# pomonam/LearnablePoolingMethods

Hardware: AMD Instinct MI355X
Metric: clips/sec training step, NetVladV1 K=256 300-frame 1152-d, bs=80, 1/2/4/8 GPU (higher is better)
Workload: dtype f32

## Files before the change

include/lpm_hip.h:

```cpp
#ifndef LPM_HIP_H
#define LPM_HIP_H

#include <stddef.h>
#include <stdint.h>

#ifdef __cplusplus
extern "C" {
#endif

#define LPM_VERSION 100

typedef void* lpm_stream_t;

enum {
    LPM_OK = 0,
    LPM_ERR_BADARG = -1,
    LPM_ERR_UNSUPPORTED_SHAPE = -2,
    LPM_ERR_WORKSPACE = -3,
    LPM_ERR_LAUNCH = -4
};

enum {
    LPM_VLAD_SOFTMAX = 1,
    LPM_VLAD_RESIDUAL = 2,
    LPM_VLAD_OUT_KMAJOR = 4,
    LPM_VLAD_NRM_RAW = 8,
    LPM_VLAD_OUT_BF16 = 16,
    LPM_VLAD_TILES_BF16 = 32,
    LPM_VLAD_NRM_BF16 = 64,
    LPM_VLAD_RAW_KMAJOR = 128,
    LPM_VLAD_DEBUG_FALLBACK = 256,
    LPM_VLAD_WIDE_ALL = 512,
    LPM_VLAD_WIDE_NONE = 1024
};

int lpm_version(void);
const char* lpm_last_error(void);

void lpm_kernel_timing_enable(int on);
int lpm_k1_forms_disable(int mask);
int lpm_kernel_timing_read(int tag, float* ms, int max);

int lpm_clock_sampler(uint64_t* out, int n, int period_ticks, lpm_stream_t stream);
int lpm_clock_marker(uint64_t* out, int slot, lpm_stream_t stream);

int lpm_l2_normalize_rows(const float* x, int64_t rows, int F, float* y, lpm_stream_t stream);

int lpm_dequantize_l2_normalize(const unsigned char* q, const int32_t* num_frames, int B, int max_frames, int F,
                                float max_quantized_value, float min_quantized_value, float* y, lpm_stream_t stream);

size_t lpm_frame_stats_workspace_bytes(int B, int S, int F);
int lpm_frame_stats(const float* raw, const int32_t* num_frames, int B, int max_frames, int F, int S,
                    float* partial, lpm_stream_t stream);
int lpm_frame_apply(const float* raw, const int32_t* num_frames, int B, int max_frames, int F, int S,
                    const float* scale, const float* shift, float* y, lpm_stream_t stream);
int lpm_frame_apply_tiles(const float* raw, const int32_t* num_frames, int B, int max_frames, int F, int S,
                          const float* scale, const float* shift, float* y, void* xt_video, int Dv, void* xt_audio, int Da,
                          lpm_stream_t stream);
int lpm_frame_apply_tiles_split(const float* raw, const int32_t* num_frames, int B, int max_frames, int F, int S, const float* scale,
                                const float* shift, float* y_video, float* y_audio, void* xt_video, int Dv, void* xt_audio, int Da,
                                lpm_stream_t stream);
int lpm_frame_bn_bwd_split(const float* dy_video, int64_t ldv, const float* dy_audio, int64_t lda, int Dv, const float* raw,
                           const int32_t* num_frames, int B, int max_frames, int F, int S, const float* mean, const float* var, float eps,
                           float* dgamma, float* dbeta, void* workspace, size_t workspace_bytes, lpm_stream_t stream);
int lpm_frame_apply_tiles2(const float* raw, const int32_t* num_frames, int B, int max_frames, int F, int S,
                           const float* scale, const float* shift, float* y, void* xt_video, void* xr_video, int Dv,
                           void* xt_audio, void* xr_audio, int Da, lpm_stream_t stream);
int lpm_frame_stats_nblk(int B, int S);
int lpm_frame_inv_norm_q8(const unsigned char* q, const int32_t* num_frames, int B, int max_frames, int F, int S,
                          float max_quantized_value, float min_quantized_value, float* inv_norm, lpm_stream_t stream);
int lpm_frame_apply_q8(const unsigned char* q, const float* inv_norm, float max_quantized_value, float min_quantized_value,
                       const int32_t* num_frames, int B, int max_frames, int F, int S, const float* scale, const float* shift, float* y,
                       lpm_stream_t stream);
int lpm_frame_apply_tiles_q8(const unsigned char* q, const float* inv_norm, float max_quantized_value, float min_quantized_value,
                             const int32_t* num_frames, int B, int max_frames, int F, int S, const float* scale, const float* shift, float* y,
                             void* xt_video, int Dv, void* xt_audio, int Da, lpm_stream_t stream);
int lpm_frame_apply_tiles_split_q8(const unsigned char* q, const float* inv_norm, float max_quantized_value, float min_quantized_value,
                                   const int32_t* num_frames, int B, int max_frames, int F, int S, const float* scale, const float* shift,
                                   float* y_video, float* y_audio, void* xt_video, int Dv, void* xt_audio, int Da, lpm_stream_t stream);
int lpm_frame_apply_tiles2_q8(const unsigned char* q, const float* inv_norm, float max_quantized_value, float min_quantized_value,
                              const int32_t* num_frames, int B, int max_frames, int F, int S, const float* scale, const float* shift, float* y,
                              void* xt_video, void* xr_video, int Dv, void* xt_audio, void* xr_audio, int Da, lpm_stream_t stream);
int lpm_frame_apply_tiles_bf16_q8(const unsigned char* q, const float* inv_norm, float max_quantized_value, float min_quantized_value,
                                  const int32_t* num_frames, int B, int max_frames, int F, int S, const float* scale, const float* shift,
                                  float* y, void* xt_video, void* xr_video, int Dv, void* xt_audio, void* xr_audio, int Da,
                                  lpm_stream_t stream);
int lpm_frame_bn_bwd(const float* dy, int64_t lddy, const float* raw, const int32_t* num_frames, int B,
                     int max_frames, int F, int S, const float* mean, const float* var, float eps, float* dgamma,
                     float* dbeta, void* workspace, size_t workspace_bytes, lpm_stream_t stream);

int lpm_bn_fold(const float* partial, int nblk, int C, int64_t rows, const float* gamma, const float* beta,
                float eps, float decay, float* mean, float* var, float* scale, float* shift,
                float* moving_mean, float* moving_var, lpm_stream_t stream);

int lpm_assign_gemm_nblk(int M);
int lpm_assign_gemm_fwd(const float* x, int64_t ldx, const float* w, int M, int D, int K, int precision,
                        float* logits, float* partial, lpm_stream_t stream);

size_t lpm_row_tiles_bytes(int B, int T, int C);
size_t lpm_weight_tiles_bytes(int R, int N);
int lpm_assign_gemm_tiles_supported(int T, int D, int K);
int lpm_assign_gemm_tiles_nblk(int B, int T);
int lpm_split_rows_tiles(const float* x, int64_t ldx, int B, int T, int C, void* out, lpm_stream_t stream);
int lpm_split_weight_tiles(const float* w, int R, int N, int transposed, void* wt, lpm_stream_t stream);
int lpm_assign_gemm_tiles_fwd(const void* xr, const void* wt, int B, int T, int D, int K, float* logits, float* partial,
                              lpm_stream_t stream);
int lpm_assign_gemm_tiles_bwd_dx(const void* dlr, const void* wtt, int B, int T, int D, int K, float* dx, int64_t lddx,
                                 lpm_stream_t stream);
int lpm_dense_tiles_fwd(const void* xr, const void* wt, int M, int Kd, int N, float* y, int64_t ldo, int form, lpm_stream_t stream);
int lpm_dense_tiles_supported(int M, int Kd, int N);
int lpm_dense_tiles_act_image_fwd(const void* xr, const void* wt, const float* bias, int M, int Kd, int N, void* out3, lpm_stream_t stream);
size_t lpm_dense_tiles_relu_bwd_workspace_bytes(int M, int N);
int lpm_dense_tiles_relu_bwd_image(const void* dyr, const void* wtt, const void* act3, int M, int Kd, int N, void* out3, float* dbias,
                                   void* workspace, size_t workspace_bytes, lpm_stream_t stream);
int lpm_image_row_tiles(const void* x3, int M, int K, int order, void* out, lpm_stream_t stream);
int lpm_skinny_weight_grad_tiles(const void* xt, const void* dyt, int R, int N1, int N2, float* dw, lpm_stream_t stream);
size_t lpm_assign_gemm_tiles_bwd_dw_workspace_bytes(int B, int T, int D, int K);
int lpm_assign_gemm_tiles_bwd_dw(const void* xt, const void* dlt, int B, int T, int D, int K, float* dw, void* workspace,
                                 size_t workspace_bytes, lpm_stream_t stream);

int lpm_vlad_aggregate_fwd(const float* assign, const float* scale, const float* shift, const float* x,
                           int64_t ldx, const float* centres, int B, int T, int D, int K, int flags,
                           float* nrm, float* asum, float* colsq, float* csq, lpm_stream_t stream);
int lpm_vlad_finalize_fwd(const float* nrm, const float* csq, int B, int D, int K, int flags, float* out,
                          float* gsq, lpm_stream_t stream);

size_t lpm_xt_bytes(int B, int T, int D);
size_t lpm_at_bytes(int B, int T, int K);
int lpm_split_frames(const float* x, int64_t ldx, int B, int T, int D, void* xt, lpm_stream_t stream);
int lpm_assign_tiles(const float* assign, const float* scale, const float* shift, int B, int T, int K, int flags,
                     void* at, lpm_stream_t stream);
int lpm_vlad_aggregate_tiles_fwd(const void* at, const void* xt, const float* centres, int B, int T, int D, int K,
                                 int flags, float* nrm, float* asum, float* colsq, float* csq, lpm_stream_t stream);

int lpm_vlad_tiles3_supported(int D, int K);
int lpm_vlad_aggregate_tiles3_fwd(const void* at, const void* xt, const float* centres, int B, int T, int D, int K,
                                  int flags, float* nrm, float* asum, float* colsq_part, lpm_stream_t stream);
int lpm_vlad_finalize2_fwd(float* nrm, const float* colsq_part, int P, int B, int D, int K, int flags, float* out,
                           float* colsq, float* csq, float* gsq, lpm_stream_t stream);
int lpm_vlad_finalize2_fwd_ld(float* nrm, const float* colsq_part, int P, int B, int D, int K, int flags, float* out,
                              int64_t out_batch_stride, float* colsq, float* csq, float* gsq, lpm_stream_t stream);

int lpm_vlad_aggregate_raw_kmajor_fwd(const void* at, const void* xt, const float* centres, int B, int T, int D, int K, int flags,
                                      float* raw_kmajor, float* asum, float* colsq_part, lpm_stream_t stream);
int lpm_vlad_row_scales(const float* colsq_part, int P, int B, int K, float* scale, float* colsq, float* csq, float* gsq,
                        lpm_stream_t stream);
int lpm_vlad_clip_slabs(int D, int K);
int lpm_vlad_aggregate_clip_kmajor_fwd(const void* at, const void* xt, const float* centres, int B, int T, int D, int K, int flags,
                                       float* raw_kmajor, float* asum, float* colsq_part, lpm_stream_t stream);
int lpm_vlad_aggregate_clip_dmajor_fwd(const void* at, const void* xt, const float* centres, int B, int T, int D, int K, int flags,
                                       float* raw_dmajor, float* asum, float* colsq_part, lpm_stream_t stream);
// ... 295 lines not shown
```

learnablepoolingmethods_amd/_capi.py:

```python
from __future__ import annotations

import ctypes as C
import os
from typing import Optional

import torch

_HERE = os.path.dirname(os.path.abspath(__file__))
LIB_PATH = os.path.join(_HERE, "_lib", "liblpm_hip.so")

LPM_VLAD_SOFTMAX = 1
LPM_VLAD_RESIDUAL = 2
LPM_VLAD_OUT_KMAJOR = 4
LPM_VLAD_NRM_RAW = 8
LPM_VLAD_OUT_BF16 = 16
LPM_VLAD_TILES_BF16 = 32
LPM_VLAD_NRM_BF16 = 64
LPM_VLAD_RAW_KMAJOR = 128
LPM_VLAD_DEBUG_FALLBACK = 256
LPM_VLAD_WIDE_ALL = 512
LPM_VLAD_WIDE_NONE = 1024

_f = C.c_void_p
_i = C.c_int
_l = C.c_int64
_s = C.c_size_t
_fl = C.c_float
SIGNATURES = {
    "lpm_version": (_i, []),
    "lpm_last_error": (C.c_char_p, []),
    "lpm_kernel_timing_enable": (None, [_i]),
    "lpm_kernel_timing_read": (_i, [_i, C.POINTER(C.c_float), _i]),
    "lpm_clock_sampler": (_i, [_f, _i, _i, _f]),
    "lpm_clock_marker": (_i, [_f, _i, _f]),
    "lpm_l2_normalize_rows": (_i, [_f, _l, _i, _f, _f]),
    "lpm_dequantize_l2_normalize": (_i, [_f, _f, _i, _i, _i, _fl, _fl, _f, _f]),
    "lpm_frame_stats_workspace_bytes": (_s, [_i, _i, _i]),
    "lpm_frame_stats": (_i, [_f, _f, _i, _i, _i, _i, _f, _f]),
    "lpm_frame_apply": (_i, [_f, _f, _i, _i, _i, _i, _f, _f, _f, _f]),
    "lpm_frame_apply_tiles": (_i, [_f, _f, _i, _i, _i, _i, _f, _f, _f, _f, _i, _f, _i, _f]),
    "lpm_frame_apply_tiles_split": (_i, [_f, _f, _i, _i, _i, _i, _f, _f, _f, _f, _f, _i, _f, _i, _f]),
    "lpm_frame_stats_nblk": (_i, [_i, _i]),
    "lpm_frame_bn_bwd": (_i, [_f, _l, _f, _f, _i, _i, _i, _i, _f, _f, _fl, _f, _f, _f, _s, _f]),
    "lpm_frame_bn_bwd_split": (_i, [_f, _l, _f, _l, _i, _f, _f, _i, _i, _i, _i, _f, _f, _fl, _f, _f, _f, _s, _f]),
    "lpm_frame_inv_norm_q8": (_i, [_f, _f, _i, _i, _i, _i, _fl, _fl, _f, _f]),
    "lpm_frame_apply_q8": (_i, [_f, _f, _fl, _fl, _f, _i, _i, _i, _i, _f, _f, _f, _f]),
    "lpm_frame_apply_tiles_q8": (_i, [_f, _f, _fl, _fl, _f, _i, _i, _i, _i, _f, _f, _f, _f, _i, _f, _i, _f]),
    "lpm_frame_apply_tiles_split_q8": (_i, [_f, _f, _fl, _fl, _f, _i, _i, _i, _i, _f, _f, _f, _f, _f, _i, _f, _i, _f]),
    "lpm_frame_apply_tiles2_q8": (_i, [_f, _f, _fl, _fl, _f, _i, _i, _i, _i, _f, _f, _f, _f, _f, _i, _f, _f, _i, _f]),
    "lpm_frame_apply_tiles_bf16_q8": (_i, [_f, _f, _fl, _fl, _f, _i, _i, _i, _i, _f, _f, _f, _f, _f, _i, _f, _f, _i, _f]),
    "lpm_bn_fold": (_i, [_f, _i, _i, _l, _f, _f, _fl, _fl, _f, _f, _f, _f, _f, _f, _f]),
    "lpm_assign_gemm_nblk": (_i, [_i]),
    "lpm_assign_gemm_fwd": (_i, [_f, _l, _f, _i, _i, _i, _i, _f, _f, _f]),
    "lpm_row_tiles_bytes": (_s, [_i, _i, _i]),
    "lpm_weight_tiles_bytes": (_s, [_i, _i]),
    "lpm_assign_gemm_tiles_supported": (_i, [_i, _i, _i]),
    "lpm_assign_gemm_tiles_nblk": (_i, [_i, _i]),
    "lpm_split_rows_tiles": (_i, [_f, _l, _i, _i, _i, _f, _f]),
    "lpm_split_weight_tiles": (_i, [_f, _i, _i, _i, _f, _f]),
    "lpm_assign_gemm_tiles_fwd": (_i, [_f, _f, _i, _i, _i, _i, _f, _f, _f]),
    "lpm_assign_gemm_tiles_bwd_dx": (_i, [_f, _f, _i, _i, _i, _i, _f, _l, _f]),
    "lpm_dense_tiles_fwd": (_i, [_f, _f, _i, _i, _i, _f, _l, _i, _f]),
    "lpm_dense_tiles_supported": (_i, [_i, _i, _i]),
    "lpm_dense_tiles_act_image_fwd": (_i, [_f, _f, _f, _i, _i, _i, _f, _f]),
    "lpm_dense_tiles_relu_bwd_workspace_bytes": (_s, [_i, _i]),
    "lpm_dense_tiles_relu_bwd_image": (_i, [_f, _f, _f, _i, _i, _i, _f, _f, _f, _s, _f]),
    "lpm_image_row_tiles": (_i, [_f, _i, _i, _i, _f, _f]),
    "lpm_skinny_weight_grad_tiles": (_i, [_f, _f, _i, _i, _i, _f, _f]),
    "lpm_assign_gemm_tiles_bwd_dw_workspace_bytes": (_s, [_i, _i, _i, _i]),
    "lpm_assign_gemm_tiles_bwd_dw": (_i, [_f, _f, _i, _i, _i, _i, _f, _f, _s, _f]),
    "lpm_vlad_aggregate_fwd": (_i, [_f, _f, _f, _f, _l, _f, _i, _i, _i, _i, _i, _f, _f, _f, _f, _f]),
    "lpm_vlad_finalize_fwd": (_i, [_f, _f, _i, _i, _i, _i, _f, _f, _f]),
    "lpm_xt_bytes": (_s, [_i, _i, _i]),
    "lpm_at_bytes": (_s, [_i, _i, _i]),
    "lpm_split_frames": (_i, [_f, _l, _i, _i, _i, _f, _f]),
    "lpm_assign_tiles": (_i, [_f, _f, _f, _i, _i, _i, _i, _f, _f]),
    "lpm_vlad_aggregate_tiles_fwd": (_i, [_f, _f, _f, _i, _i, _i, _i, _i, _f, _f, _f, _f, _f]),
    "lpm_vlad_tiles3_supported": (_i, [_i, _i]),
    "lpm_vlad_aggregate_tiles3_fwd": (_i, [_f, _f, _f, _i, _i, _i, _i, _i, _f, _f, _f, _f]),
    "lpm_vlad_finalize2_fwd_ld": (_i, [_f, _f, _i, _i, _i, _i, _i, _f, _l, _f, _f, _f, _f]),
    "lpm_vlad_finalize2_fwd": (_i, [_f, _f, _i, _i, _i, _i, _i, _f, _f, _f, _f, _f]),
    "lpm_proj_supported": (_i, [_i, _l, _i]),
    "lpm_proj_fwd_workspace_bytes": (_s, [_i, _l, _i]),
    "lpm_proj_fwd": (_i, [_f, _l, _f, _i, _l, _i, _f, _f, _s, _f]),
    "lpm_proj_fwd_parts": (_i, [_f, _l, _l, _i, _f, _i, _f, _l, _f, _i, _l, _i, _f, _f, _s, _f]),
    "lpm_split_weight_tiles_parts": (_i, [_f, _l, _l, _i, _f, _i, _f, _l, _i, _l, _f, _f]),
    "lpm_proj_dx": (_i, [_f, _f, _i, _l, _i, _f, _l, _f]),
    "lpm_proj_fwd_parts_w16": (_i, [_f, _l, _l, _f, _i, _f, _l, _f, _i, _l, _i, _f, _f, _s, _f]),
    "lpm_proj_dx_w16": (_i, [_f, _f, _i, _l, _i, _f, _l, _f]),
    "lpm_frame_tiles_bf16_bytes": (_s, [_i, _i, _i]),
    "lpm_frame_steps_bf16": (_i, [_i]),
    "lpm_frame_apply_tiles2": (_i, [_f, _f, _i, _i, _i, _i, _f, _f, _f, _f, _f, _i, _f, _f, _i, _f]),
    "lpm_frame_apply_tiles_bf16": (_i, [_f, _f, _i, _i, _i, _i, _f, _f, _f, _f, _f, _i, _f, _f, _i, _f]),
    "lpm_split_weight_tiles_bf16": (_i, [_f, _i, _i, _i, _f, _f]),
    "lpm_split_frames_bf16": (_i, [_f, _l, _i, _i, _i, _f, _f]),
    "lpm_assign_gemm_tiles_fwd_bf16": (_i, [_f, _f, _i, _i, _i, _i, _f, _f, _f]),
    "lpm_k1_forms_disable": (_i, [_i]),
    "lpm_mha_bwd_set_terms": (_i, [_i]),
    "lpm_assign_gemm_tiles_bwd_dw_bf16": (_i, [_f, _f, _i, _i, _i, _i, _f, _f, _s, _f]),
    "lpm_assign_tiles_bf16": (_i, [_f, _f, _f, _i, _i, _i, _i, _f, _f]),
    "lpm_vlad_aggregate_tiles3_fwd_bf16": (_i, [_f, _f, _f, _i, _i, _i, _i, _i, _f, _f, _f, _f]),
    "lpm_vlad_clip16_slabs": (_i, [_i, _i]),
    "lpm_vlad_aggregate_clip_fwd_bf16": (_i, [_f, _f, _f, _i, _i, _i, _i, _i, _f, _f, _f, _f]),
    "lpm_vlad_aggregate_raw_kmajor_fwd": (_i, [_f, _f, _f, _i, _i, _i, _i, _i, _f, _f, _f, _f]),
    "lpm_vlad_smx_stats_bytes": (_s, [_i, _i]),
    "lpm_vlad_smx_supported": (_i, [_i, _i, _i]),
    "lpm_vlad_aggregate_raw_kmajor_smx_fwd": (_i, [_f, _f, _f, _f, _f, _i, _i, _i, _i, _i, _f, _f, _f, _f, _f]),
    "lpm_vlad_row_scales": (_i, [_f, _i, _i, _i, _f, _f, _f, _f, _f]),
    "lpm_vlad_clip_slabs": (_i, [_i, _i]),
    "lpm_vlad_aggregate_clip_kmajor_fwd": (_i, [_f, _f, _f, _i, _i, _i, _i, _i, _f, _f, _f, _f]),
    "lpm_vlad_aggregate_clip_dmajor_fwd": (_i, [_f, _f, _f, _i, _i, _i, _i, _i, _f, _f, _f, _f]),
    "lpm_vlad_kmajor_workspace_bytes": (_s, [_i, _i, _i]),
    "lpm_vlad_aggregate_kmajor_scaled_fwd": (_i, [_f, _f, _f, _i, _i, _i, _i, _i, _f, _f, _f, _f, _f, _f, _f, _s, _f]),
    "lpm_split_rows_scaled": (_i, [_f, _l, _l, _i, _f, _f, _f]),
    "lpm_layer_norm_act_fwd_rs": (_i, [_f, _f, _i, _f, _f, _f, _f, _i, _i, _i, _fl, _f, _l, _f, _f, _f, _s, _f]),
    "lpm_layer_norm_act_image_fwd": (_i, [_f, _f, _i, _f, _f, _f, _f, _i, _i, _i, _fl, _f, _l, _f, _f, _f, _f, _s, _f]),
    "lpm_vlad_fused_supported": (_i, [_i, _i]),
    "lpm_vlad_fused_workspace_bytes": (_s, [_i, _i, _i]),
    "lpm_vlad_aggregate_fused_fwd": (_i, [_f, _f, _f, _i, _i, _i, _i, _i, _f, _f, _f, _f, _f, _f, _f, _s, _f]),
    "lpm_vlad_bwd_workspace_bytes": (_s, [_i, _i, _i]),
    "lpm_vlad_aggregate_bwd": (_i, [_f, _f, _f, _f, _f, _f, _f, _f, _f, _f, _l, _f, _i, _i, _i, _i, _i, _f, _f, _l,
                                    _i, _f, _f, _s, _f]),
    "lpm_vlad_bwd_tiles_workspace_bytes": (_s, [_i, _i, _i, _i]),
    "lpm_vlad_aggregate_bwd_tiles_ld": (_i, [_f, _l, _f, _f, _f, _f, _f, _f, _f, _f, _f, _f, _i, _i, _i, _i, _i, _f, _f, _f, _f, _s, _f]),
    "lpm_vlad_aggregate_bwd_tiles": (_i, [_f, _f, _f, _f, _f, _f, _f, _f, _f, _f, _f, _i, _i, _i, _i, _i, _f, _f, _f, _f, _s, _f]),
    "lpm_input_bn_grads": (_i, [_f, _f, _f, _f, _f, _f, _f, _f, _i, _i, _i, _f, _f, _f]),
    "lpm_vlad_aggregate_bwd_tiles_dx": (_i, [_f, _s, _f, _f, _i, _i, _i, _i, _f, _l, _i, _f]),
    "lpm_bn_rows_workspace_bytes": (_s, [_i, _i]),
# ... 145 lines not shown
```

learnablepoolingmethods_amd/csrc/frame_prep.hip:

```cpp
#include "lpm_common.h"

namespace lpm {

constexpr int FP_ROWS = 32;

__device__ __forceinline__ int sample_index(int j, float step, int nf) {
    const float v = __fmul_rn((float)j, step);
    return (int)__fmul_rn(fminf(v, 1.0f), (float)nf);
}

__device__ __forceinline__ float dequant_row_inv_norm(const uchar4* __restrict__ src, int lane, int F4, float scalar, float bias,
                                                      float4 (&v)[8]) {
    float ss = 0.f;
#pragma unroll
    for (int i = 0; i < 8; ++i) {
        const int c = lane + 64 * i;
        v[i] = make_float4(0.f, 0.f, 0.f, 0.f);
        if (c < F4) {
            const uchar4 u = src[c];
            v[i] = make_float4(fmaf((float)u.x, scalar, bias), fmaf((float)u.y, scalar, bias), fmaf((float)u.z, scalar, bias),
                               fmaf((float)u.w, scalar, bias));
        }
        ss += v[i].x * v[i].x + v[i].y * v[i].y + v[i].z * v[i].z + v[i].w * v[i].w;
    }
    ss = wave_sum(ss);
    return rsqrtf(fmaxf(ss, 1e-12f));
}

template <typename T>
struct FrameSrc;
template <>
struct FrameSrc<float> {
    const float* __restrict__ raw;
    __device__ __forceinline__ float4 load4(int64_t off, int64_t) const { return *reinterpret_cast<const float4*>(raw + off); }
};
template <>
struct FrameSrc<unsigned char> {
    const unsigned char* __restrict__ raw;
    const float* __restrict__ inv;
    float scalar, bias;
    __device__ __forceinline__ float4 load4(int64_t off, int64_t row) const {
        const float s = inv[row];
        if (s == 0.f) return make_float4(0.f, 0.f, 0.f, 0.f);
        const uchar4 u = *reinterpret_cast<const uchar4*>(raw + off);
        return make_float4(__fmul_rn(fmaf((float)u.x, scalar, bias), s), __fmul_rn(fmaf((float)u.y, scalar, bias), s),
                           __fmul_rn(fmaf((float)u.z, scalar, bias), s), __fmul_rn(fmaf((float)u.w, scalar, bias), s));
    }
};

__global__ __launch_bounds__(256) void frame_stats_kernel(const float* __restrict__ raw,
                                                          const int32_t* __restrict__ num_frames, int B,
                                                          int max_frames, int F, int S, float step,
                                                          float* __restrict__ partial) {
    const int r0 = blockIdx.x * FP_ROWS;
    const int rows = B * S;
    const int r1 = min(rows, r0 + FP_ROWS);
    __shared__ int64_t base[FP_ROWS];
    if (threadIdx.x < FP_ROWS) {
        const int r = r0 + threadIdx.x;
        if (r < rows) {
            const int b = r / S, j = r % S;
            int idx = sample_index(j, step, num_frames[b]);
            idx = max(0, min(idx, max_frames - 1));
            base[threadIdx.x] = ((int64_t)b * max_frames + idx) * F;
        }
    }
    __syncthreads();
    for (int c = threadIdx.x; c < F; c += 256) {
        float s = 0.f, q = 0.f;
        for (int r = 0; r < r1 - r0; ++r) {
            const float v = raw[base[r] + c];
            s += v;
            q = fmaf(v, v, q);
        }
        float* p = partial + (int64_t)blockIdx.x * 2 * F;
        p[c] = s;
        p[F + c] = q;
    }
}

template <typename Src>
__global__ __launch_bounds__(256) void frame_apply_kernel(Src raw, const int32_t* __restrict__ num_frames, int B,
                                                          int max_frames, int F, int S, float step,
                                                          const float* __restrict__ scale,
                                                          const float* __restrict__ shift, float* __restrict__ y) {
    const int F4 = F / 4;
    const int64_t total = (int64_t)B * S * F4;
    for (int64_t i = (int64_t)blockIdx.x * 256 + threadIdx.x; i < total; i += (int64_t)gridDim.x * 256) {
        const int r = (int)(i / F4), c = (int)(i % F4) * 4;
        const int b = r / S, j = r % S;
        int idx = sample_index(j, step, num_frames[b]);
        idx = max(0, min(idx, max_frames - 1));
        float4 v = raw.load4(((int64_t)b * max_frames + idx) * F + c, r);
        if (scale) {
            const float4 sc = *reinterpret_cast<const float4*>(scale + c);
            const float4 sh = *reinterpret_cast<const float4*>(shift + c);
            v.x = fmaf(v.x, sc.x, sh.x); v.y = fmaf(v.y, sc.y, sh.y);
            v.z = fmaf(v.z, sc.z, sh.z); v.w = fmaf(v.w, sc.w, sh.w);
        }
        *reinterpret_cast<float4*>(y + (int64_t)r * F + c) = v;
    }
}

__device__ __forceinline__ unsigned fp_bf16_rne(float v) {
    unsigned u = __float_as_uint(v);
    u += 0x7fffu + ((u >> 16) & 1u);
    return u >> 16;
}
template <typename Src>
__global__ __launch_bounds__(256) void frame_apply_tiles_kernel(Src raw, const int32_t* __restrict__ num_frames, int B,
                                                                int max_frames, int F, int S, float step,
                                                                const float* __restrict__ scale,
                                                                const float* __restrict__ shift, float* __restrict__ y,
                                                                uint4* __restrict__ xtv, int Dv,
                                                                uint4* __restrict__ xta, int Da, float* __restrict__ y2) {
    const int F4 = F / 4, NS = (S + 15) / 16;
    const int64_t total = (int64_t)B * NS * 2 * F4;
    for (int64_t w = (int64_t)blockIdx.x * 256 + threadIdx.x; w < total; w += (int64_t)gridDim.x * 256) {
        const int c4 = (int)(w % F4);
        const int64_t r = w / F4;
        const int kh = (int)(r & 1), st = (int)((r >> 1) % NS), b = (int)((r >> 1) / NS);
        const int c = 4 * c4;
        float4 sc = make_float4(1.f, 1.f, 1.f, 1.f), sh = make_float4(0.f, 0.f, 0.f, 0.f);
        if (scale) {
            sc = *reinterpret_cast<const float4*>(scale + c);
            sh = *reinterpret_cast<const float4*>(shift + c);
        }
        const int nf = num_frames[b];
        float v[4][8];
#pragma unroll
        for (int e = 0; e < 8; ++e) {
            const int j = 16 * st + 8 * kh + e;
            float4 f = make_float4(0.f, 0.f, 0.f, 0.f);
            if (j < S) {
                int idx = sample_index(j, step, nf);
                idx = max(0, min(idx, max_frames - 1));
                f = raw.load4(((int64_t)b * max_frames + idx) * F + c, (int64_t)b * S + j);
                f.x = fmaf(f.x, sc.x, sh.x); f.y = fmaf(f.y, sc.y, sh.y);
                f.z = fmaf(f.z, sc.z, sh.z); f.w = fmaf(f.w, sc.w, sh.w);
                const int64_t row = (int64_t)b * S + j;
                if (!y2) *reinterpret_cast<float4*>(y + row * F + c) = f;
                else if (c < Dv) *reinterpret_cast<float4*>(y + row * Dv + c) = f;
                else *reinterpret_cast<float4*>(y2 + row * Da + (c - Dv)) = f;
            }
            v[0][e] = f.x; v[1][e] = f.y; v[2][e] = f.z; v[3][e] = f.w;
        }
        uint4* xt = (c < Dv) ? xtv : xta;
        const int DT = ((c < Dv) ? Dv : Da) / 32;
        const int cb = (c < Dv) ? c : c - Dv;
        if (xt == nullptr) continue;
#pragma unroll
        for (int q = 0; q < 4; ++q) {
            unsigned h[8], l[8];
#pragma unroll
            for (int e = 0; e < 8; ++e) {
                h[e] = fp_bf16_rne(v[q][e]);
                l[e] = fp_bf16_rne(v[q][e] - __uint_as_float(h[e] << 16));
            }
            const int d = cb + q, dt = d >> 5, jj = d & 31;
            const int64_t base = ((((int64_t)b * NS + st) * DT + dt) * 2) * 64 + kh * 32 + jj;
// ... 116 lines not shown
            if (c < F4) dst[c] = make_float4(v[i].x * inv, v[i].y * inv, v[i].z * inv, v[i].w * inv);
        }
    }
}

template <int PL, typename Src>
__global__ __launch_bounds__(256) void frame_apply_tiles_bf16_kernel(Src raw, const int32_t* __restrict__ num_frames,
                                                                     int B, int max_frames, int F, int S, float step,
                                                                     const float* __restrict__ scale, const float* __restrict__ shift,
                                                                     float* __restrict__ y, uint4* __restrict__ xtv, uint4* __restrict__ xrv,
                                                                     int Dv, uint4* __restrict__ xta, uint4* __restrict__ xra, int Da) {
    const int F8 = F / 8, NSP = 4 * ((S + 63) / 64), MT = NSP / 2;
    const int64_t total = (int64_t)B * NSP * 2 * F8;
    for (int64_t w = (int64_t)blockIdx.x * 256 + threadIdx.x; w < total; w += (int64_t)gridDim.x * 256) {
        const int c8 = (int)(w % F8);
        const int64_t r = w / F8;
        const int kh = (int)(r & 1), st = (int)((r >> 1) % NSP), b = (int)((r >> 1) / NSP);
        const int c = 8 * c8;
        float sc[8], sh[8];
#pragma unroll
        for (int q = 0; q < 8; ++q) {
            sc[q] = scale ? scale[c + q] : 1.f;
            sh[q] = scale ? shift[c + q] : 0.f;
        }
        const int nf = num_frames[b];
        float v[8][8];
#pragma unroll
        for (int e = 0; e < 8; ++e) {
            const int j = 16 * st + 8 * kh + e;
            float4 f0 = make_float4(0.f, 0.f, 0.f, 0.f), f1 = f0;
            if (j < S) {
                int idx = sample_index(j, step, nf);
                idx = max(0, min(idx, max_frames - 1));
                const int64_t src = ((int64_t)b * max_frames + idx) * F + c, row = (int64_t)b * S + j;
                f0 = raw.load4(src, row);
                f1 = raw.load4(src + 4, row);
                f0.x = fmaf(f0.x, sc[0], sh[0]); f0.y = fmaf(f0.y, sc[1], sh[1]); f0.z = fmaf(f0.z, sc[2], sh[2]); f0.w = fmaf(f0.w, sc[3], sh[3]);
                f1.x = fmaf(f1.x, sc[4], sh[4]); f1.y = fmaf(f1.y, sc[5], sh[5]); f1.z = fmaf(f1.z, sc[6], sh[6]); f1.w = fmaf(f1.w, sc[7], sh[7]);
                if (y) {
                    float* dst = y + ((int64_t)b * S + j) * F + c;
                    *reinterpret_cast<float4*>(dst) = f0;
                    *reinterpret_cast<float4*>(dst + 4) = f1;
                }
            }
            v[e][0] = f0.x; v[e][1] = f0.y; v[e][2] = f0.z; v[e][3] = f0.w; v[e][4] = f1.x; v[e][5] = f1.y; v[e][6] = f1.z; v[e][7] = f1.w;
        }
        const bool video = c < Dv;
        uint4* xt = video ? xtv : xta;
        uint4* xr = video ? xrv : xra;
        if (xt == nullptr) continue;
        const int Dn = video ? Dv : Da, cb = video ? c : c - Dv;
        unsigned h[8][8], l[8][8];
#pragma unroll
        for (int e = 0; e < 8; ++e)
#pragma unroll
            for (int q = 0; q < 8; ++q) {
                h[e][q] = fp_bf16_rne(v[e][q]);
                if (PL == 2) l[e][q] = fp_bf16_rne(v[e][q] - __uint_as_float(h[e][q] << 16));
            }
        const int DT = Dn / 32, CS = Dn / 16;
        const int NSF = PL == 2 ? (S + 15) / 16 : NSP;
        if (st < NSF) {
#pragma unroll
            for (int q = 0; q < 8; ++q) {
                const int d = cb + q;
                const int64_t base = ((((int64_t)b * NSF + st) * DT + (d >> 5)) * PL) * 64 + kh * 32 + (d & 31);
                xt[base] = make_uint4(h[0][q] | (h[1][q] << 16), h[2][q] | (h[3][q] << 16), h[4][q] | (h[5][q] << 16), h[6][q] | (h[7][q] << 16));
                if (PL == 2)
                    xt[base + 64] = make_uint4(l[0][q] | (l[1][q] << 16), l[2][q] | (l[3][q] << 16), l[4][q] | (l[5][q] << 16), l[6][q] | (l[7][q] << 16));
            }
        }
        if (xr == nullptr) continue;
#pragma unroll
        for (int e = 0; e < 8; ++e) {
            const int j = 16 * st + 8 * kh + e;
            const int64_t base = ((((int64_t)b * MT + (j >> 5)) * CS + (cb >> 4)) * PL) * 64 + ((cb >> 3) & 1) * 32 + (j & 31);
            xr[base] = make_uint4(h[e][0] | (h[e][1] << 16), h[e][2] | (h[e][3] << 16), h[e][4] | (h[e][5] << 16), h[e][6] | (h[e][7] << 16));
            if (PL == 2)
                xr[base + 64] = make_uint4(l[e][0] | (l[e][1] << 16), l[e][2] | (l[e][3] << 16), l[e][4] | (l[e][5] << 16), l[e][6] | (l[e][7] << 16));
        }
    }
}

}

static inline int fp_nblk(int B, int S) { return (B * S + lpm::FP_ROWS - 1) / lpm::FP_ROWS; }

extern "C" size_t lpm_frame_stats_workspace_bytes(int B, int S, int F) {
    return (size_t)fp_nblk(B, S) * 2 * F * sizeof(float);
}
extern "C" int lpm_frame_stats_nblk(int B, int S) { return fp_nblk(B, S); }

#define LPM_FRAME_CHECK(name)                                                                                       \
    LPM_REQUIRE(raw && num_frames, LPM_ERR_BADARG, name ": null pointer");                                          \
    LPM_REQUIRE(B > 0 && max_frames > 0 && F > 0 && S > 0, LPM_ERR_BADARG, name ": bad sizes");                      \
    LPM_REQUIRE(F % 4 == 0, LPM_ERR_UNSUPPORTED_SHAPE, name ": need F %% 4 == 0 (F=%d)", F)

#define LPM_FRAME_Q8_CHECK(name)                                                                                                     \
    LPM_REQUIRE(q && inv_norm && num_frames, LPM_ERR_BADARG, name ": null pointer");                                                 \
    LPM_REQUIRE(max_quantized_value > min_quantized_value, LPM_ERR_BADARG, name ": empty quantisation range");                       \
    LPM_REQUIRE(B > 0 && max_frames > 0 && F > 0 && S > 0, LPM_ERR_BADARG, name ": bad sizes");                                       \
    LPM_REQUIRE(F % 4 == 0 && ((uintptr_t)q & 3) == 0, LPM_ERR_UNSUPPORTED_SHAPE, name ": need F %% 4 == 0, aligned input (F=%d)", F)

namespace {

using lpm::FrameSrc;

FrameSrc<unsigned char> q8_src(const unsigned char* q, const float* inv_norm, float max_quantized_value, float min_quantized_value) {
    const float range = max_quantized_value - min_quantized_value;
    return FrameSrc<unsigned char>{q, inv_norm, range / 255.0f, range / 512.0f + min_quantized_value};
}

template <typename Src>
int launch_frame_apply(Src raw, const int32_t* num_frames, int B, int max_frames, int F, int S, const float* scale, const float* shift,
                       float* y, hipStream_t stream, const char* name) {
    using namespace lpm;
    LPM_REQUIRE(y && ((scale == nullptr) == (shift == nullptr)), LPM_ERR_BADARG, "%s: bad pointers", name);
    const float step = 1.0f / (float)S;
    const int64_t total = (int64_t)B * S * (F / 4);
    const int64_t want = (total + 255) / 256;
    hipLaunchKernelGGL(frame_apply_kernel<Src>, dim3((unsigned)(want < 4096 ? want : 4096)), dim3(256), 0, stream, raw, num_frames, B,
                       max_frames, F, S, step, scale, shift, y);
    return check_launch(name);
}

template <typename Src>
int launch_frame_apply_tiles(Src raw, const int32_t* num_frames, int B, int max_frames, int F, int S, const float* scale,
                             const float* shift, float* y, float* y2, void* xt_video, int Dv, void* xt_audio, int Da, hipStream_t stream,
                             const char* name) {
    using namespace lpm;
    if (y2 == nullptr) {
        LPM_REQUIRE(y && ((scale == nullptr) == (shift == nullptr)), LPM_ERR_BADARG, "%s: bad pointers", name);
        LPM_REQUIRE(Dv > 0 && Da >= 0 && Dv + Da == F && Dv % 32 == 0 && Da % 32 == 0, LPM_ERR_UNSUPPORTED_SHAPE,
                    "%s: need Dv + Da == F, both multiples of 32 (F=%d Dv=%d Da=%d)", name, F, Dv, Da);
    } else {
        LPM_REQUIRE(y && ((scale == nullptr) == (shift == nullptr)), LPM_ERR_BADARG, "%s: bad pointers", name);
        LPM_REQUIRE(Dv > 0 && Da > 0 && Dv + Da == F && Dv % 32 == 0 && Da % 32 == 0 && (((uintptr_t)y | (uintptr_t)y2) & 15) == 0,
                    LPM_ERR_UNSUPPORTED_SHAPE, "%s: need Dv + Da == F, both multiples of 32, aligned outputs (F=%d Dv=%d Da=%d)", name, F,
                    Dv, Da);
    }
    const float step = 1.0f / (float)S;
    const int64_t total = (int64_t)B * ((S + 15) / 16) * 2 * (F / 4);
    const int64_t want = (total + 255) / 256;
    hipLaunchKernelGGL(frame_apply_tiles_kernel<Src>, dim3((unsigned)(want < 8192 ? want : 8192)), dim3(256), 0, stream, raw, num_frames,
                       B, max_frames, F, S, step, scale, shift, y, (uint4*)xt_video, Dv, (uint4*)xt_audio, Da, y2);
    return check_launch(name);
}

template <int PL, typename Src>
int launch_frame_apply_tiles_bf16(Src raw, const int32_t* num_frames, int B, int max_frames, int F, int S, const float* scale,
                                  const float* shift, float* y, void* xt_video, void* xr_video, int Dv, void* xt_audio, void* xr_audio,
                                  int Da, hipStream_t stream, const char* name) {
    using namespace lpm;
    if (PL == 1)
        LPM_REQUIRE(xt_video && xr_video && ((scale == nullptr) == (shift == nullptr)) && ((xt_audio == nullptr) == (xr_audio == nullptr)),
                    LPM_ERR_BADARG, "%s: bad pointers", name);
    else
        LPM_REQUIRE(y && xt_video && ((scale == nullptr) == (shift == nullptr)) && (Da == 0 || xt_audio), LPM_ERR_BADARG,
                    "%s: bad pointers", name);
    LPM_REQUIRE(Dv > 0 && Da >= 0 && Dv + Da == F && Dv % 32 == 0 && Da % 32 == 0, LPM_ERR_UNSUPPORTED_SHAPE,
                "%s: need Dv + Da == F, both multiples of 32 (F=%d Dv=%d Da=%d)", name, F, Dv, Da);
    const float step = 1.0f / (float)S;
    const int64_t total = (int64_t)B * 4 * ((S + 63) / 64) * 2 * (F / 8);
    const int64_t want = (total + 255) / 256;
    hipLaunchKernelGGL((frame_apply_tiles_bf16_kernel<PL, Src>), dim3((unsigned)(want < 16384 ? want : 16384)), dim3(256), 0, stream, raw,
                       num_frames, B, max_frames, F, S, step, scale, shift, y, (uint4*)xt_video, (uint4*)xr_video, Dv, (uint4*)xt_audio,
                       (uint4*)xr_audio, Da);
    return check_launch(name);
}

}

extern "C" int lpm_frame_stats(const float* raw, const int32_t* num_frames, int B, int max_frames, int F, int S,
                               float* partial, lpm_stream_t stream) {
    using namespace lpm;
    LPM_FRAME_CHECK("lpm_frame_stats");
    LPM_REQUIRE(partial, LPM_ERR_BADARG, "lpm_frame_stats: null workspace");
    const float step = 1.0f / (float)S;
    hipLaunchKernelGGL(frame_stats_kernel, dim3(fp_nblk(B, S)), dim3(256), 0, (hipStream_t)stream, raw, num_frames, B,
                       max_frames, F, S, step, partial);
    return check_launch("lpm_frame_stats");
}

extern "C" int lpm_frame_apply(const float* raw, const int32_t* num_frames, int B, int max_frames, int F, int S,
                               const float* scale, const float* shift, float* y, lpm_stream_t stream) {
    LPM_FRAME_CHECK("lpm_frame_apply");
    return launch_frame_apply(FrameSrc<float>{raw}, num_frames, B, max_frames, F, S, scale, shift, y, (hipStream_t)stream, "lpm_frame_apply");
}

extern "C" int lpm_frame_apply_tiles(const float* raw, const int32_t* num_frames, int B, int max_frames, int F, int S,
                                     const float* scale, const float* shift, float* y, void* xt_video, int Dv,
                                     void* xt_audio, int Da, lpm_stream_t stream) {
    LPM_FRAME_CHECK("lpm_frame_apply_tiles");
    return launch_frame_apply_tiles(FrameSrc<float>{raw}, num_frames, B, max_frames, F, S, scale, shift, y, nullptr, xt_video, Dv, xt_audio,
                                    Da, (hipStream_t)stream, "lpm_frame_apply_tiles");
}
extern "C" int lpm_frame_apply_tiles_split(const float* raw, const int32_t* num_frames, int B, int max_frames, int F, int S,
                                           const float* scale, const float* shift, float* y_video, float* y_audio, void* xt_video, int Dv,
                                           void* xt_audio, int Da, lpm_stream_t stream) {
    LPM_FRAME_CHECK("lpm_frame_apply_tiles_split");
    LPM_REQUIRE(y_video && y_audio, LPM_ERR_BADARG, "lpm_frame_apply_tiles_split: bad pointers");
    return launch_frame_apply_tiles(FrameSrc<float>{raw}, num_frames, B, max_frames, F, S, scale, shift, y_video, y_audio, xt_video, Dv,
                                    xt_audio, Da, (hipStream_t)stream, "lpm_frame_apply_tiles_split");
}

extern "C" size_t lpm_frame_tiles_bf16_bytes(int B, int S, int D) { return (size_t)B * 4 * ((S + 63) / 64) * (D / 32) * 1024; }
extern "C" int lpm_frame_apply_tiles_bf16(const float* raw, const int32_t* num_frames, int B, int max_frames, int F, int S,
                                          const float* scale, const float* shift, float* y, void* xt_video, void* xr_video, int Dv,
                                          void* xt_audio, void* xr_audio, int Da, lpm_stream_t stream) {
    LPM_FRAME_CHECK("lpm_frame_apply_tiles_bf16");
    return launch_frame_apply_tiles_bf16<1>(FrameSrc<float>{raw}, num_frames, B, max_frames, F, S, scale, shift, y, xt_video, xr_video, Dv,
                                            xt_audio, xr_audio, Da, (hipStream_t)stream, "lpm_frame_apply_tiles_bf16");
}

extern "C" int lpm_frame_apply_tiles2(const float* raw, const int32_t* num_frames, int B, int max_frames, int F, int S,
                                      const float* scale, const float* shift, float* y, void* xt_video, void* xr_video, int Dv,
                                      void* xt_audio, void* xr_audio, int Da, lpm_stream_t stream) {
    LPM_FRAME_CHECK("lpm_frame_apply_tiles2");
    return launch_frame_apply_tiles_bf16<2>(FrameSrc<float>{raw}, num_frames, B, max_frames, F, S, scale, shift, y, xt_video, xr_video, Dv,
                                            xt_audio, xr_audio, Da, (hipStream_t)stream, "lpm_frame_apply_tiles2");
}

extern "C" int lpm_frame_inv_norm_q8(const unsigned char* q, const int32_t* num_frames, int B, int max_frames, int F, int S,
                                     float max_quantized_value, float min_quantized_value, float* inv_norm, lpm_stream_t stream) {
    using namespace lpm;
    LPM_FRAME_Q8_CHECK("lpm_frame_inv_norm_q8");
    LPM_REQUIRE(F <= 2048, LPM_ERR_UNSUPPORTED_SHAPE, "lpm_frame_inv_norm_q8: need F <= 2048 (F=%d)", F);
    const FrameSrc<unsigned char> src = q8_src(q, inv_norm, max_quantized_value, min_quantized_value);
    const int64_t rows = (int64_t)B * S, want = (rows + 3) / 4;
    hipLaunchKernelGGL(frame_inv_norm_q8_kernel, dim3((unsigned)(want < 16384 ? want : 16384)), dim3(256), 0, (hipStream_t)stream, q,
                       num_frames, B, max_frames, F, S, 1.0f / (float)S, src.scalar, src.bias, inv_norm);
    return check_launch("lpm_frame_inv_norm_q8");
}

extern "C" int lpm_frame_apply_q8(const unsigned char* q, const float* inv_norm, float max_quantized_value, float min_quantized_value,
                                  const int32_t* num_frames, int B, int max_frames, int F, int S, const float* scale, const float* shift,
                                  float* y, lpm_stream_t stream) {
    LPM_FRAME_Q8_CHECK("lpm_frame_apply_q8");
    return launch_frame_apply(q8_src(q, inv_norm, max_quantized_value, min_quantized_value), num_frames, B, max_frames, F, S, scale, shift,
                              y, (hipStream_t)stream, "lpm_frame_apply_q8");
}

extern "C" int lpm_frame_apply_tiles_q8(const unsigned char* q, const float* inv_norm, float max_quantized_value,
                                        float min_quantized_value, const int32_t* num_frames, int B, int max_frames, int F, int S,
                                        const float* scale, const float* shift, float* y, void* xt_video, int Dv, void* xt_audio, int Da,
                                        lpm_stream_t stream) {
    LPM_FRAME_Q8_CHECK("lpm_frame_apply_tiles_q8");
    return launch_frame_apply_tiles(q8_src(q, inv_norm, max_quantized_value, min_quantized_value), num_frames, B, max_frames, F, S, scale,
                                    shift, y, nullptr, xt_video, Dv, xt_audio, Da, (hipStream_t)stream, "lpm_frame_apply_tiles_q8");
}

extern "C" int lpm_frame_apply_tiles_split_q8(const unsigned char* q, const float* inv_norm, float max_quantized_value,
                                              float min_quantized_value, const int32_t* num_frames, int B, int max_frames, int F, int S,
                                              const float* scale, const float* shift, float* y_video, float* y_audio, void* xt_video,
                                              int Dv, void* xt_audio, int Da, lpm_stream_t stream) {
    LPM_FRAME_Q8_CHECK("lpm_frame_apply_tiles_split_q8");
    LPM_REQUIRE(y_video && y_audio, LPM_ERR_BADARG, "lpm_frame_apply_tiles_split_q8: bad pointers");
    return launch_frame_apply_tiles(q8_src(q, inv_norm, max_quantized_value, min_quantized_value), num_frames, B, max_frames, F, S, scale,
                                    shift, y_video, y_audio, xt_video, Dv, xt_audio, Da, (hipStream_t)stream, "lpm_frame_apply_tiles_split_q8");
}

extern "C" int lpm_frame_apply_tiles_bf16_q8(const unsigned char* q, const float* inv_norm, float max_quantized_value,
                                             float min_quantized_value, const int32_t* num_frames, int B, int max_frames, int F, int S,
                                             const float* scale, const float* shift, float* y, void* xt_video, void* xr_video, int Dv,
                                             void* xt_audio, void* xr_audio, int Da, lpm_stream_t stream) {
    LPM_FRAME_Q8_CHECK("lpm_frame_apply_tiles_bf16_q8");
    return launch_frame_apply_tiles_bf16<1>(q8_src(q, inv_norm, max_quantized_value, min_quantized_value), num_frames, B, max_frames, F, S,
                                            scale, shift, y, xt_video, xr_video, Dv, xt_audio, xr_audio, Da, (hipStream_t)stream,
                                            "lpm_frame_apply_tiles_bf16_q8");
}

extern "C" int lpm_frame_apply_tiles2_q8(const unsigned char* q, const float* inv_norm, float max_quantized_value,
                                         float min_quantized_value, const int32_t* num_frames, int B, int max_frames, int F, int S,
                                         const float* scale, const float* shift, float* y, void* xt_video, void* xr_video, int Dv,
                                         void* xt_audio, void* xr_audio, int Da, lpm_stream_t stream) {
    LPM_FRAME_Q8_CHECK("lpm_frame_apply_tiles2_q8");
    return launch_frame_apply_tiles_bf16<2>(q8_src(q, inv_norm, max_quantized_value, min_quantized_value), num_frames, B, max_frames, F, S,
                                            scale, shift, y, xt_video, xr_video, Dv, xt_audio, xr_audio, Da, (hipStream_t)stream,
                                            "lpm_frame_apply_tiles2_q8");
}

extern "C" int lpm_frame_bn_bwd(const float* dy, int64_t lddy, const float* raw, const int32_t* num_frames, int B,
                                int max_frames, int F, int S, const float* mean, const float* var, float eps,
                                float* dgamma, float* dbeta, void* workspace, size_t workspace_bytes,
                                lpm_stream_t stream) {
    using namespace lpm;
    LPM_FRAME_CHECK("lpm_frame_bn_bwd");
    LPM_REQUIRE(dy && mean && var && dgamma && dbeta && workspace && lddy >= F, LPM_ERR_BADARG, "lpm_frame_bn_bwd: bad pointers");
    LPM_REQUIRE(workspace_bytes >= lpm_frame_stats_workspace_bytes(B, S, F), LPM_ERR_WORKSPACE, "lpm_frame_bn_bwd: workspace too small");
    const float step = 1.0f / (float)S;
    const int nblk = fp_nblk(B, S);
    hipStream_t s = (hipStream_t)stream;
    hipLaunchKernelGGL(frame_bn_bwd_partial_kernel, dim3(nblk), dim3(256), 0, s, dy, lddy, raw, num_frames, B, max_frames, F, S,
                       step, (float*)workspace, (const float*)nullptr, (int64_t)0, F);
    hipLaunchKernelGGL(frame_bn_bwd_reduce_kernel, dim3((F + 15) / 16), dim3(1024), 0, s, (const float*)workspace, nblk, F, mean,
                       var, eps, dgamma, dbeta);
    return check_launch("lpm_frame_bn_bwd");
}
extern "C" int lpm_frame_bn_bwd_split(const float* dy_video, int64_t ldv, const float* dy_audio, int64_t lda, int Dv, const float* raw,
                                      const int32_t* num_frames, int B, int max_frames, int F, int S, const float* mean, const float* var,
                                      float eps, float* dgamma, float* dbeta, void* workspace, size_t workspace_bytes, lpm_stream_t stream) {
    using namespace lpm;
    LPM_FRAME_CHECK("lpm_frame_bn_bwd_split");
// ... 39 lines not shown
```

learnablepoolingmethods_amd/csrc/mha_x3.hip:

```cpp
#include "lpm_common.h"
#include "operand_format.h"
#include <atomic>
#include <cstdlib>

namespace lpm {

constexpr float MX_LOG2E = 1.4426950408889634f;
constexpr float MX_LN2 = 0.6931471805599453f;
typedef __bf16 mx_bf16x8 __attribute__((ext_vector_type(8)));
typedef __bf16 mx_bf16x2 __attribute__((ext_vector_type(2)));
typedef float mx_f32x2 __attribute__((ext_vector_type(2)));
typedef unsigned mx_u32x4 __attribute__((ext_vector_type(4)));

__device__ __forceinline__ f32x4 mx_mfma(mx_u32x4 a, mx_u32x4 b, f32x4 c) {
    return __builtin_amdgcn_mfma_f32_16x16x32_bf16(__builtin_bit_cast(mx_bf16x8, a), __builtin_bit_cast(mx_bf16x8, b), c, 0, 0, 0);
}
__device__ __forceinline__ void mx_split2(float a, float b, unsigned& hi, unsigned& lo) {
    const mx_f32x2 v = {a, b};
    const mx_bf16x2 h = __builtin_convertvector(v, mx_bf16x2);
    const mx_f32x2 hf = __builtin_convertvector(h, mx_f32x2);
    const mx_bf16x2 l = __builtin_convertvector(v - hf, mx_bf16x2);
    hi = __builtin_bit_cast(unsigned, h);
    lo = __builtin_bit_cast(unsigned, l);
}
// ... 285 lines not shown
            oa = mx_mfma(vl, ph, oa);
        }
        sum += __shfl_xor(sum, 16, 64);
        sum += __shfl_xor(sum, 32, 64);
        const float inv = 1.f / sum;
        if (qrow < L) {
            if (4 * g < D)
                mx_store_act4(o, (int64_t)b * L + qrow, ldo, hh * D + 4 * g, oimg, (oa[0] + ob[0]) * inv, (oa[1] + ob[1]) * inv,
                              (oa[2] + ob[2]) * inv, (oa[3] + ob[3]) * inv, im, vmax);
            if (g == 0) lse[((int64_t)b * h + hh) * L + qrow] = m * MX_LN2 + __logf(sum);
        }
    }
    if (oimg) of_amax_commit(im.oamax, vmax);
}

constexpr int MX_DQ_NT = 512;
template <int NKT, bool AFFINE, int D, bool RAGGED>
__global__ __launch_bounds__(MX_DQ_NT) void mha_bwd_dq_x3_kernel(const float* __restrict__ q, const float* __restrict__ k,
                                                            const float* __restrict__ v, int64_t ld, const float* __restrict__ o,
                                                            const float* __restrict__ dout, int64_t ldo,
                                                            const float* __restrict__ lse, int L, int h, float scale,
                                                            const float* __restrict__ key_scale, const float* __restrict__ key_shift,
                                                            float* __restrict__ dq, int64_t ldd, const float* __restrict__ corr_a,
                                                            const float* __restrict__ corr_b, int img, int oimg, const MxImg im) {
    extern __shared__ __attribute__((aligned(16))) unsigned char smem[];
    float vmax = 0.f;
    constexpr int LP = NKT * 16;
    const int nkt = (L + 15) >> 4;
    const float qmul = AFFINE ? scale : scale * MX_LOG2E;
    unsigned char* Kp = smem;
    unsigned char* Vp = Kp + mx_rowplanes_bytes(LP, D);
    unsigned char* Kt = Vp + mx_rowplanes_bytes(LP, D);
    float* ksc = reinterpret_cast<float*>(Kt + mx_tplanes_bytes(LP));
    float* ksh = ksc + LP;
    float* cas = ksh + LP;
    float* cbs = cas + LP;
    const int tid = threadIdx.x, lane = tid & 63, wave = tid >> 6;
    const int l15 = lane & 15, g = lane >> 4;
    const int lid = xcd_remap(blockIdx.x, gridDim.x);
    const int b = lid / h, hh = lid % h;
    const int TS = mx_tstride(LP);

    if (RAGGED || D < 16) {
        for (int i = tid; i < (2 * mx_rowplanes_bytes(LP, D) + mx_tplanes_bytes(LP)) / 16; i += MX_DQ_NT)
            reinterpret_cast<mx_u32x4*>(smem)[i] = mx_u32x4{0u, 0u, 0u, 0u};
        __syncthreads();
    }
    if (AFFINE) {
        for (int i = tid; i < LP; i += MX_DQ_NT) {
            ksc[i] = (i < L) ? key_scale[i] : 1.f;
            ksh[i] = (i < L) ? key_shift[i] : 0.f;
            cas[i] = (corr_a && i < L) ? corr_a[i] : 0.f;
            cbs[i] = (corr_b && i < L) ? corr_b[i] : 0.f;
        }
    }
    mx_stage_rows<D>(Kp, k, ld, b, L, LP, hh, 1.f, tid, MX_DQ_NT);
    mx_stage_rows<D>(Vp, v, ld, b, L, LP, hh, 1.f, tid, MX_DQ_NT);
    mx_stage_transposed<D>(Kt, k, ld, b, L, LP, hh, tid, MX_DQ_NT);
    __syncthreads();

#pragma unroll 1
    for (int qt = wave; qt < nkt; qt += MX_DQ_NT / 64) {
        const int qrow = qt * 16 + l15;
        const bool qok = qrow < L;
        mx_u32x4 qh = {0u, 0u, 0u, 0u}, ql = qh, gh = qh, gl = qh;
        float dpart = 0.f;
        if (qok) {
            const int c0 = hh * D + ((D == 16) ? 8 * (g & 1) : 0);
            const float* qp = q + ((int64_t)b * L + qrow) * ld + c0;
            const float4 a = *reinterpret_cast<const float4*>(qp), c = *reinterpret_cast<const float4*>(qp + 4);
            const float qv[8] = {a.x * qmul, a.y * qmul, a.z * qmul, a.w * qmul, c.x * qmul, c.y * qmul, c.z * qmul, c.w * qmul};
            mx_split8(qv, qh, ql);
            const int64_t off = ((int64_t)b * L + qrow) * ldo + c0;
            const float4 ga = *reinterpret_cast<const float4*>(dout + off), gc = *reinterpret_cast<const float4*>(dout + off + 4);
            float4 oa, oc;
            mx_load_o8(o, (int64_t)b * L + qrow, ldo, c0, oimg, oa, oc, im);
            const float gv[8] = {ga.x, ga.y, ga.z, ga.w, gc.x, gc.y, gc.z, gc.w};
            mx_split8(gv, gh, gl);
            dpart = ga.x * oa.x + ga.y * oa.y + ga.z * oa.z + ga.w * oa.w + gc.x * oc.x + gc.y * oc.y + gc.z * oc.z + gc.w * oc.w;
        }
        if (D == 16) dpart += __shfl_xor(dpart, 16, 64);
        const float dqv = dpart;
        const float lq = qok ? lse[((int64_t)b * h + hh) * L + qrow] * MX_LOG2E : INFINITY;
        mx_u32x4 qb1, qb2, gb1, gb2;
        mx_col_frags<D>(qh, ql, g, qb1, qb2);
        mx_col_frags<D>(gh, gl, g, gb1, gb2);
        f32x4 dqa = {0.f, 0.f, 0.f, 0.f}, dqb = {0.f, 0.f, 0.f, 0.f};
#pragma unroll 2
        for (int j = 0; j < NKT / 2; ++j) {
            float ds8[8];
#pragma unroll
            for (int t = 0; t < 2; ++t) {
                const int kt = 2 * j + t;
                const mx_u32x4 ka = mx_row_frag<D>(Kp, LP, kt, l15, g), va = mx_row_frag<D>(Vp, LP, kt, l15, g);
                f32x4 st = {0.f, 0.f, 0.f, 0.f}, dp = {0.f, 0.f, 0.f, 0.f};
                st = mx_mfma(ka, qb1, st);
                dp = mx_mfma(va, gb1, dp);
                if (D == 16) {
                    st = mx_mfma(ka, qb2, st);
                    dp = mx_mfma(va, gb2, dp);
                }
                float z[4];
#pragma unroll
                for (int r = 0; r < 4; ++r) {
                    z[r] = st[r];
                    if (AFFINE) z[r] = fmaf(st[r], ksc[kt * 16 + 4 * g + r], ksh[kt * 16 + 4 * g + r]) * MX_LOG2E;
                }
                if (RAGGED) {
#pragma unroll
                    for (int r = 0; r < 4; ++r)
                        if (kt * 16 + 4 * g + r >= L) z[r] = -INFINITY;
                }
#pragma unroll
                for (int r = 0; r < 4; ++r) {
                    const float pr = __builtin_amdgcn_exp2f(z[r] - lq);
                    float dsv = pr * (dp[r] - dqv);
                    if (AFFINE) {
                        const int key = kt * 16 + 4 * g + r;
                        dsv = dsv * ksc[key] - cas[key] - st[r] * cbs[key];
                    }
                    ds8[4 * t + r] = dsv;
                }
            }
            mx_u32x4 dh, dl;
            mx_split8(ds8, dh, dl);
            const unsigned char* kc = Kt + l15 * TS + (32 * j + 8 * g) * 2;
            const mx_u32x4 kh = *reinterpret_cast<const mx_u32x4*>(kc), kl = *reinterpret_cast<const mx_u32x4*>(kc + 16 * TS);
            dqa = mx_mfma(kh, dh, dqa);
            dqb = mx_mfma(kh, dl, dqb);
            dqa = mx_mfma(kl, dh, dqa);
        }
        if (qok && 4 * g < D)
            mx_store_grad4(dq, ((int64_t)b * L + qrow) * ldd + hh * D + 4 * g, img, (dqa[0] + dqb[0]) * scale, (dqa[1] + dqb[1]) * scale,
                           (dqa[2] + dqb[2]) * scale, (dqa[3] + dqb[3]) * scale, im, vmax);
    }
    if (img) of_amax_commit(im.gamax, vmax);
}

#ifndef LPM_DKV_NT_LONG
#define LPM_DKV_NT_LONG 1024
#endif
__host__ __device__ constexpr int mx_dkv_nt(int nkt) { return nkt >= 20 ? LPM_DKV_NT_LONG : 512; }
template <int NKT, bool AFFINE, int D, bool CORR = true>
__global__ __launch_bounds__(mx_dkv_nt(NKT)) void mha_bwd_dkv_x3_kernel(const float* __restrict__ q, const float* __restrict__ k,
                                                             const float* __restrict__ v, int64_t ld, const float* __restrict__ o,
                                                             const float* __restrict__ dout, int64_t ldo,
                                                             const float* __restrict__ lse, int L, int h, float scale,
                                                             const float* __restrict__ key_scale, const float* __restrict__ key_shift,
                                                             float* __restrict__ dk, float* __restrict__ dv, int64_t ldd,
                                                             const float* __restrict__ corr_a, const float* __restrict__ corr_b,
                                                             float* __restrict__ dz_partial, int img, int oimg, const MxImg im) {
    extern __shared__ __attribute__((aligned(16))) unsigned char smem[];
    float vmax = 0.f;
    constexpr int LP = NKT * 16;
    constexpr int MX_DKV_NT = mx_dkv_nt(NKT);
    constexpr int NH = D / 8;
    const int nkt = (L + 15) >> 4;
    const float qmul = AFFINE ? scale : scale * MX_LOG2E;
    unsigned char* Qp = smem;
    unsigned char* Gp = Qp + mx_rowplanes_bytes(LP, D);
    unsigned char* Qt = Gp + mx_rowplanes_bytes(LP, D);
    unsigned char* Gt = Qt + mx_tplanes_bytes(LP);
    float* lses = reinterpret_cast<float*>(Gt + mx_tplanes_bytes(LP));
    float* Dq = lses + LP;
    const bool stats_only = (dk == nullptr);
    const int tid = threadIdx.x, lane = tid & 63, wave = tid >> 6;
    const int l15 = lane & 15, g = lane >> 4;
    const int lid = xcd_remap(blockIdx.x, gridDim.x);
    const int b = lid / h, hh = lid % h;
    const int TS = mx_tstride(LP);

    if (L != LP || D < 16) {
        for (int i = tid; i < (2 * mx_rowplanes_bytes(LP, D) + 2 * mx_tplanes_bytes(LP)) / 16; i += MX_DKV_NT)
            reinterpret_cast<mx_u32x4*>(smem)[i] = mx_u32x4{0u, 0u, 0u, 0u};
    }
    for (int i = tid; i < LP; i += MX_DKV_NT) {
        lses[i] = (i < L) ? lse[((int64_t)b * h + hh) * L + i] * MX_LOG2E : INFINITY;
        Dq[i] = 0.f;
    }
    __syncthreads();
    for (int i0 = 0; i0 < L * NH; i0 += MX_DKV_NT) {
        const int i = i0 + tid;
        float part = 0.f;
        int row = 0;
        if (i < L * NH) {
            row = i / NH;
            const int hf = i % NH;
            const float* qp = q + ((int64_t)b * L + row) * ld + hh * D + 8 * hf;
            const int64_t off = ((int64_t)b * L + row) * ldo + hh * D + 8 * hf;
            const float4 qa = *reinterpret_cast<const float4*>(qp), qc = *reinterpret_cast<const float4*>(qp + 4);
            const float4 ga = *reinterpret_cast<const float4*>(dout + off), gc = *reinterpret_cast<const float4*>(dout + off + 4);
            float4 oa, oc;
            mx_load_o8(o, (int64_t)b * L + row, ldo, hh * D + 8 * hf, oimg, oa, oc, im);
            part = ga.x * oa.x + ga.y * oa.y + ga.z * oa.z + ga.w * oa.w + gc.x * oc.x + gc.y * oc.y + gc.z * oc.z + gc.w * oc.w;
            const float qv[8] = {qa.x * qmul, qa.y * qmul, qa.z * qmul, qa.w * qmul, qc.x * qmul, qc.y * qmul, qc.z * qmul, qc.w * qmul};
            const float gv[8] = {ga.x, ga.y, ga.z, ga.w, gc.x, gc.y, gc.z, gc.w};
            mx_u32x4 qh, ql, gh, gl;
            mx_split8(qv, qh, ql);
            mx_split8(gv, gh, gl);
            *reinterpret_cast<mx_u32x4*>(Qp + ((0 * NH + hf) * LP + row) * 16) = qh;
            *reinterpret_cast<mx_u32x4*>(Qp + ((1 * NH + hf) * LP + row) * 16) = ql;
            *reinterpret_cast<mx_u32x4*>(Gp + ((0 * NH + hf) * LP + row) * 16) = gh;
            *reinterpret_cast<mx_u32x4*>(Gp + ((1 * NH + hf) * LP + row) * 16) = gl;
            const int pos = mx_perm(row);
#pragma unroll
            for (int e = 0; e < 8; ++e) {
                const int dd = 8 * hf + e, sh = (e & 1) * 16;
                *reinterpret_cast<unsigned short*>(Qt + dd * TS + pos * 2) = (unsigned short)(qh[e >> 1] >> sh);
                *reinterpret_cast<unsigned short*>(Qt + 16 * TS + dd * TS + pos * 2) = (unsigned short)(ql[e >> 1] >> sh);
                *reinterpret_cast<unsigned short*>(Gt + dd * TS + pos * 2) = (unsigned short)(gh[e >> 1] >> sh);
                *reinterpret_cast<unsigned short*>(Gt + 16 * TS + dd * TS + pos * 2) = (unsigned short)(gl[e >> 1] >> sh);
            }
        }
        if (NH == 2) part += __shfl_xor(part, 1, 64);
        if (i < L * NH && (i % NH) == 0) Dq[row] = part;
    }
    __syncthreads();

#pragma unroll 1
    for (int kt = wave; kt < nkt; kt += MX_DKV_NT / 64) {
        const int krow = kt * 16 + l15;
        const bool kok = krow < L;
        mx_u32x4 kh = {0u, 0u, 0u, 0u}, kl = kh, vh = kh, vl = kh;
        if (kok) {
            const int64_t off = ((int64_t)b * L + krow) * ld + hh * D + ((D == 16) ? 8 * (g & 1) : 0);
            const float4 ka = *reinterpret_cast<const float4*>(k + off), kc = *reinterpret_cast<const float4*>(k + off + 4);
            const float4 va = *reinterpret_cast<const float4*>(v + off), vc = *reinterpret_cast<const float4*>(v + off + 4);
            const float kv[8] = {ka.x, ka.y, ka.z, ka.w, kc.x, kc.y, kc.z, kc.w};
            const float vv[8] = {va.x, va.y, va.z, va.w, vc.x, vc.y, vc.z, vc.w};
            mx_split8(kv, kh, kl);
            mx_split8(vv, vh, vl);
        }
        mx_u32x4 kb1, kb2, vb1, vb2;
        mx_col_frags<D>(kh, kl, g, kb1, kb2);
        mx_col_frags<D>(vh, vl, g, vb1, vb2);
        const float sck = (key_scale && kok) ? key_scale[krow] : 1.f, shk = (key_shift && kok) ? key_shift[krow] : 0.f;
        const float cak = (corr_a && kok) ? corr_a[krow] : 0.f, cbk = (corr_b && kok) ? corr_b[krow] : 0.f;
        f32x4 dka = {0.f, 0.f, 0.f, 0.f}, dkb = dka, dva = dka, dvb = dka;
        float zs = 0.f, zq = 0.f;
#pragma unroll 2
        for (int j = 0; j < NKT / 2; ++j) {
            float p8[8], ds8[8];
#pragma unroll
            for (int t = 0; t < 2; ++t) {
                const int qt = 2 * j + t;
                const mx_u32x4 qa = mx_row_frag<D>(Qp, LP, qt, l15, g), ga = mx_row_frag<D>(Gp, LP, qt, l15, g);
                f32x4 st = {0.f, 0.f, 0.f, 0.f}, dp = {0.f, 0.f, 0.f, 0.f};
                st = mx_mfma(qa, kb1, st);
                dp = mx_mfma(ga, vb1, dp);
                if (D == 16) {
                    st = mx_mfma(qa, kb2, st);
                    dp = mx_mfma(ga, vb2, dp);
                }
                const float4 lq4v = *reinterpret_cast<const float4*>(lses + qt * 16 + 4 * g);
                const float4 dq4v = *reinterpret_cast<const float4*>(Dq + qt * 16 + 4 * g);
                const float lq4[4] = {lq4v.x, lq4v.y, lq4v.z, lq4v.w}, dq4[4] = {dq4v.x, dq4v.y, dq4v.z, dq4v.w};
#pragma unroll
                for (int r = 0; r < 4; ++r) {
                    const int qr = qt * 16 + 4 * g + r;
                    const float sraw = st[r];
                    float z = sraw;
                    if (AFFINE) z = fmaf(sraw, sck, shk) * MX_LOG2E;
                    if (!kok) z = -INFINITY;
                    const float pr = __builtin_amdgcn_exp2f(z - lq4[r]);
                    const float dz = pr * (dp[r] - dq4[r]);
                    float dsv = dz;
                    if (AFFINE) {
                        zs += dz;
                        zq = fmaf(dz, sraw, zq);
                        if constexpr (CORR) dsv = (qr < L) ? dz * sck - cak - sraw * cbk : 0.f;
                        else dsv = (qr < L) ? dz * sck : 0.f;
                    }
                    p8[4 * t + r] = pr;
                    ds8[4 * t + r] = dsv;
                }
            }
            if (!stats_only) {
                mx_u32x4 ph, pl, dh, dl;
                mx_split8(p8, ph, pl);
                mx_split8(ds8, dh, dl);
                const int offt = l15 * TS + (32 * j + 8 * g) * 2;
                const mx_u32x4 gth = *reinterpret_cast<const mx_u32x4*>(Gt + offt), gtl = *reinterpret_cast<const mx_u32x4*>(Gt + 16 * TS + offt);
                const mx_u32x4 qth = *reinterpret_cast<const mx_u32x4*>(Qt + offt), qtl = *reinterpret_cast<const mx_u32x4*>(Qt + 16 * TS + offt);
                dva = mx_mfma(gth, ph, dva);
                dvb = mx_mfma(gth, pl, dvb);
                dva = mx_mfma(gtl, ph, dva);
                dka = mx_mfma(qth, dh, dka);
                dkb = mx_mfma(qth, dl, dkb);
                dka = mx_mfma(qtl, dh, dka);
            }
        }
        if (!stats_only && kok && 4 * g < D) {
            const int64_t off = ((int64_t)b * L + krow) * ldd + hh * D + 4 * g;
            const float kmul = AFFINE ? 1.f : MX_LN2;
            mx_store_dk4(dk, (int64_t)b * L + krow, ldd, hh * D + 4 * g, img, (dka[0] + dkb[0]) * kmul, (dka[1] + dkb[1]) * kmul, (dka[2] + dkb[2]) * kmul, (dka[3] + dkb[3]) * kmul, im, vmax);
            mx_store_grad4(dv, off, img, dva[0] + dvb[0], dva[1] + dvb[1], dva[2] + dvb[2], dva[3] + dvb[3], im, vmax);
        }
        if (dz_partial) {
            zs += __shfl_xor(zs, 16, 64); zs += __shfl_xor(zs, 32, 64);
            zq += __shfl_xor(zq, 16, 64); zq += __shfl_xor(zq, 32, 64);
            if (g == 0 && kok) {
                float* out = dz_partial + ((int64_t)b * h + hh) * 2 * L;
                out[krow] = zs;
                out[L + krow] = zq;
            }
        }
    }
    if (img) of_amax_commit(im.gamax, vmax);
}

template <int NKT, int TPW, bool DKV> __host__ __device__ constexpr int mx_h_nt() {
    constexpr int w = (NKT + TPW - 1) / TPW;
    return TPW == 1 ? (DKV ? mx_dkv_nt(NKT) : MX_DQ_NT) : (w <= 4 ? 256 : (w >= 16 ? 1024 : 64 * w));
}
template <int NKT, bool AFFINE, int D, bool RAGGED, int TPW>
__global__ __launch_bounds__((mx_h_nt<NKT, TPW, false>())) void mha_bwd_dq_h_kernel(const float* __restrict__ q, const float* __restrict__ k,
                                                            const float* __restrict__ v, int64_t ld, const float* __restrict__ o,
                                                            const float* __restrict__ dout, int64_t ldo,
                                                            const float* __restrict__ lse, int L, int h, float scale,
                                                            const float* __restrict__ key_scale, const float* __restrict__ key_shift,
                                                            float* __restrict__ dq, int64_t ldd, const float* __restrict__ corr_a,
                                                            const float* __restrict__ corr_b, int img, int oimg, const MxImg im) {
    extern __shared__ __attribute__((aligned(16))) unsigned char smem[];
    float vmax = 0.f;
    constexpr int LP = NKT * 16;
    constexpr int NT = mx_h_nt<NKT, TPW, false>();
    const int nkt = (L + 15) >> 4;
    const float qmul = AFFINE ? scale : scale * MX_LOG2E;
    unsigned char* Kp = smem;
    unsigned char* Vp = Kp + mx_rowplanes_bytes(LP, D);
    unsigned char* Kt = Vp + mx_rowplanes_bytes(LP, D);
    float* ksc = reinterpret_cast<float*>(Kt + mx_tplanes_bytes(LP));
    float* ksh = ksc + LP;
    float* cas = ksh + LP;
    float* cbs = cas + LP;
    const int tid = threadIdx.x, lane = tid & 63, wave = tid >> 6;
    const int l15 = lane & 15, g = lane >> 4;
    const int lid = xcd_remap(blockIdx.x, gridDim.x);
    const int b = lid / h, hh = lid % h;
    const int TS = mx_tstride(LP);

    if (RAGGED || D < 16) {
        for (int i = tid; i < (2 * mx_rowplanes_bytes(LP, D) + mx_tplanes_bytes(LP)) / 16; i += NT)
            reinterpret_cast<mx_u32x4*>(smem)[i] = mx_u32x4{0u, 0u, 0u, 0u};
        __syncthreads();
    }
    if (AFFINE) {
        for (int i = tid; i < LP; i += NT) {
// ... 735 lines not shown
```

learnablepoolingmethods_amd/frame_level_models.py:

```python
from __future__ import annotations

import contextlib
import math

import torch

from . import FLAGS, layers, model_utils, models, ops, transformer_utils, video_level_models, video_pooling_modules
from . import variables as vs


class NetVLAD():

    residual = True

    def __init__(self, feature_size, max_frames, cluster_size, add_batch_norm, is_training, scope_id=None):
        self.feature_size = feature_size
        self.max_frames = max_frames
        self.is_training = is_training
        self.add_batch_norm = add_batch_norm
        self.cluster_size = int(cluster_size)

    def forward(self, reshaped_input, kmajor=False, input_affine=None, storage="f32", lazy=False, out_slot=None):
        D, K, dev = self.feature_size, self.cluster_size, reshaped_input.device
        std = 1 / math.sqrt(D)
# ... 11 lines not shown
                           is_training=self.is_training, kmajor=kmajor, input_affine=input_affine, storage=storage, lazy=lazy,
                           out_slot=out_slot)


class LightVLAD(NetVLAD):
    residual = False


def _project_gate_classify(vlad, vocab_size, cluster_size, hidden1_size, add_batch_norm, relu, gating, remove_diag,
                           is_training, **unused_params):
    parts = vlad if isinstance(vlad, tuple) else None
    dev = parts[0].device if parts else vlad.device
    vlad_dim = sum(p.shape[1] for p in parts if p is not None) if parts else vlad.shape[1]
    hidden1_weights = vs.get_variable("hidden1_weights", [vlad_dim, hidden1_size],
                                      vs.random_normal_initializer(1 / math.sqrt(cluster_size)), device=dev)
    if parts and ops.projection_parts_ok(getattr(parts[0], "_lpm_raw", parts[0]), ops.row_scale_of(parts[0]),
                                         getattr(parts[0], "_lpm_scale_ks", 0), parts[1], hidden1_weights):
        activation = ops.projection_parts(parts[0], parts[1], hidden1_weights)
    else:
        if parts:
            vlad = ops.materialise(parts[0])
            vlad = torch.cat([vlad, parts[1]], 1) if parts[1] is not None else vlad
        activation = ops.projection(vlad, hidden1_weights) if vlad.is_cuda else vlad.matmul(hidden1_weights)
    small = is_training and ops.bn_small_ok(activation)
    if add_batch_norm and relu and small:
        activation = ops.bn_small(activation, *layers.bn_variables("hidden1_bn", hidden1_size, dev), act=1)
    elif add_batch_norm and relu:
        activation = layers.batch_norm(activation, is_training, "hidden1_bn")
    else:
        hidden1_biases = vs.get_variable("hidden1_biases", [hidden1_size], vs.random_normal_initializer(0.01), device=dev)
        activation = activation + hidden1_biases
    if relu and not (add_batch_norm and small):
        activation = torch.clamp(activation, 0.0, 6.0)
    if gating:
        gating_weights = vs.get_variable("gating_weights_2", [hidden1_size, hidden1_size],
                                         vs.random_normal_initializer(1 / math.sqrt(hidden1_size)), device=dev)
        gates = activation.matmul(gating_weights)
        if remove_diag:
            gates = gates - torch.diagonal(gating_weights) * activation
        if not add_batch_norm:
            raise NotImplementedError("context gating without batch norm is broken in the reference (App. C12)")
        if small:
            activation = ops.bn_small(gates, *layers.bn_variables("gating_bn", hidden1_size, dev), act=2, mul=activation)
        else:
            gates = layers.batch_norm(gates, is_training, "gating_bn")
            activation = activation * torch.sigmoid(gates)
    vs.summary("activation", activation)
    aggregated_model = getattr(video_level_models, "MoeModel")
    return aggregated_model().create_model(model_input=activation, vocab_size=vocab_size, is_training=is_training,
                                           **unused_params)


class _GammaWatch:
    EVERY, FLOOR = 8, 0.2

    def __init__(self):
        self.disabled, self.count, self.pending, self.host = False, 0, None, None

    def ok(self, gamma):
        if self.disabled:
            return False
        if self.count == 0:
            self._decide(float(gamma.detach().abs().min()))
        elif self.pending is not None and self.pending.query():
            self.pending = None
            self._decide(float(self.host))
        if not self.disabled and self.pending is None and self.count % self.EVERY == 0 and self.count > 0:
            if self.host is None:
                self.host = torch.empty((), dtype=torch.float32).pin_memory()
            self.host.copy_(gamma.detach().abs().min(), non_blocking=True)
            self.pending = torch.cuda.Event()
            self.pending.record()
        self.count += 1
        return not self.disabled

    def _decide(self, min_abs_gamma):
        if not (min_abs_gamma >= self.FLOOR):
            import warnings
            self.disabled = True
            warnings.warn(f"input_bn: min |gamma| = {min_abs_gamma:.3g} < {self.FLOOR}: the closed-form gamma / beta gradients are "
                          "switched off, the input gradient is formed explicitly from now on")


def _sample_and_normalise(model_input, num_frames, iterations, add_batch_norm, is_training, storage="f32"):
    bn = layers.bn_variables("input_bn", model_input.shape[2], model_input.device) if add_batch_norm else (None,) * 4
    return ops.frame_sample_bn(model_input, num_frames.reshape(-1), iterations, *bn, is_training=is_training, storage=storage,
                               materialize=storage == "f32" or vs.default_store().summaries is not None)


class NetVladV1(models.BaseModel):

    def create_model(self, model_input, vocab_size, num_frames, iterations=None, add_batch_norm=None,
                     sample_random_frames=None, cluster_size=None, hidden_size=None, is_training=True, encoder=None,
                     **unused_params):
        iterations = iterations or FLAGS.iterations
        add_batch_norm = add_batch_norm or FLAGS.netvlad_add_batch_norm
        cluster_size = cluster_size or FLAGS.netvlad_cluster_size
        hidden1_size = hidden_size or FLAGS.netvlad_hidden_size
        relu, gating, remove_diag = FLAGS.netvlad_relu, FLAGS.gating, FLAGS.gating_remove_diag
        encoder = FLAGS.netvlad_encoder if encoder is None else encoder
        storage = FLAGS.netvlad_storage
        if storage == "bf16" and (encoder or not add_batch_norm or not model_input.is_cuda):
            raise ValueError("netvlad_storage='bf16' is the gated-NetVLAD configuration: netvlad_encoder off, batch norm on, on the GPU")

        max_frames, feature_size = iterations, model_input.shape[2]
        has_audio = feature_size > 1024
        shortcut = False
        if (FLAGS.input_bn_grad_shortcut and add_batch_norm and is_training and model_input.is_cuda and torch.is_grad_enabled()
                and ops.netvlad_input_shortcut_ok(max_frames, 1024, cluster_size)
                and (not has_audio or ops.netvlad_input_shortcut_ok(max_frames, 128, cluster_size // 4))):
            g_in, b_in, _, _ = layers.bn_variables("input_bn", feature_size, model_input.device)
            watch = getattr(g_in, "_lpm_gamma_watch", None)
            if watch is None:
                watch = g_in._lpm_gamma_watch = _GammaWatch()
            shortcut = watch.ok(g_in)
        if storage == "bf16" and is_training and torch.is_grad_enabled() and not shortcut:
            if not getattr(NetVladV1, "_warned_bf16_fallback", False):
                import warnings
                NetVladV1._warned_bf16_fallback = True
                warnings.warn("netvlad_storage='bf16': the closed-form input_bn gradients are unavailable; training steps fall "
                              "back to fp32 storage (explicit input-gradient path)")
            storage = "f32"

        reshaped_input = _sample_and_normalise(model_input, num_frames, iterations, add_batch_norm, is_training, storage)
        if storage == "f32" or vs.default_store().summaries is not None:
            vs.summary("input_bn", reshaped_input)

        video_NetVLAD = NetVLAD(1024, max_frames, cluster_size, add_batch_norm, is_training, "netvlad_rgb_scope")
        audio_NetVLAD = NetVLAD(128, max_frames, cluster_size // 4, add_batch_norm, is_training, "netvlad_audio_scope")
        aff_v = aff_a = None
        if shortcut:
            with torch.no_grad():
                rgb, audio = reshaped_input[:, 0:1024], reshaped_input[:, 1024:]
            if ops.SPLIT_VECTOR and g_in.is_cuda and g_in.dim() == 1 and g_in.shape[0] > 1024:
                (gv, ga), (bv, ba) = ops.split_vector(g_in, 1024), ops.split_vector(b_in, 1024)
                aff_v, aff_a = (gv, bv), (ga, ba)
            else:
                aff_v, aff_a = (g_in[0:1024], b_in[0:1024]), (g_in[1024:], b_in[1024:])
        if aff_v is not None:
            pass
        elif has_audio and reshaped_input.is_cuda:
            rgb, audio = ops.split_columns(reshaped_input, 1024)
        else:
            rgb, audio = reshaped_input[:, 0:1024], reshaped_input[:, 1024:]
        use_side = has_audio and reshaped_input.is_cuda and FLAGS.audio_side_stream
        side = ops.side_stream(audio, reshaped_input) if use_side else contextlib.nullcontext()
        video_encoder_block = None
        if encoder:
            video_encoder_block = transformer_utils.TransformerEncoder(
                feature_size=1024, hidden_size=1024, num_heads=64, attention_dropout=0.1, ff_filter_size=4 * 1024,
                ff_relu_dropout=0.1, is_train=is_training, scope_id="encode1")
        batch = model_input.shape[0]
        lazy_v = bool(encoder and FLAGS.netvlad_lazy_descriptor and storage == "f32" and reshaped_input.is_cuda
                      and (aff_v is not None or not torch.is_grad_enabled())
                      and video_encoder_block.fused_shape(batch, cluster_size, True) and ops.netvlad_lazy_ok(max_frames, 1024, cluster_size))
        slots = None
        lazy5 = bool(storage == "bf16" and not encoder and has_audio and FLAGS.netvlad_lazy_descriptor and FLAGS.descriptor_slots
                     and aff_v is not None and batch <= 128 and hidden1_size % 512 == 0 and cluster_size % 32 == 0)
        if lazy5:
            slots = ops.DescriptorSlots(batch, [(1, 128 * (cluster_size // 4))], reshaped_input)
        elif (storage == "bf16" and not encoder and has_audio and FLAGS.descriptor_slots and aff_v is not None):
            slots = ops.DescriptorSlots(batch, [(1, 1024 * cluster_size), (1, 128 * (cluster_size // 4))], reshaped_input)
        with vs.variable_scope("video_VLAD"):
            vlad_video = video_NetVLAD.forward(rgb, kmajor=encoder, input_affine=aff_v, storage=storage, lazy=lazy_v or lazy5,
                                               out_slot=slots.slots[0] if slots and not lazy5 else None)
            if vs.default_store().summaries is not None:
                vs.summary("vlad_video", ops.materialise(vlad_video))
        if has_audio:
            with side, vs.variable_scope("audio_VLAD"):
                vlad_audio = audio_NetVLAD.forward(audio, kmajor=encoder, input_affine=aff_a, storage=storage,
                                                   out_slot=(slots.slots[0 if lazy5 else 1] if slots else None))
                vs.summary("vlad_audio", vlad_audio)

        if encoder:
            if has_audio:
                with vs.variable_scope("audio_attention"):
                    audio_encoder_block = transformer_utils.TransformerEncoder(
                        feature_size=128, hidden_size=128, num_heads=16, attention_dropout=0.1, ff_filter_size=4 * 128,
                        ff_relu_dropout=0.1, is_train=is_training, scope_id="encode2")
                if FLAGS.descriptor_slots and video_encoder_block.fused(vlad_video) and audio_encoder_block.fused(vlad_audio):
                    slots = ops.DescriptorSlots(vlad_video.shape[0], [(cluster_size, 1024), (cluster_size // 4, 128)], vlad_video)
            with vs.variable_scope("video_attention"):
                vlad_video = video_encoder_block.forward(vlad_video, out_slot=slots.slots[0] if slots else None)
            if has_audio:
                with side, vs.variable_scope("audio_attention"):
                    vlad_audio = audio_encoder_block.forward(vlad_audio, out_slot=slots.slots[1] if slots else None)
            if slots is None:
                vlad_video = vlad_video.reshape(-1, 1024 * cluster_size)
                if has_audio:
                    vlad_audio = vlad_audio.reshape(-1, 128 * (cluster_size // 4))
        if use_side:
            side.join(vlad_audio)

        if lazy5:
            if vs.default_store().summaries is not None:
                vs.summary("vlad", torch.cat([ops.materialise(vlad_video), vlad_audio.reshape(batch, -1)], 1))
            return _project_gate_classify((vlad_video, vlad_audio.reshape(batch, -1)), vocab_size, cluster_size, hidden1_size,
                                          add_batch_norm, relu, gating, remove_diag, is_training, **unused_params)
        if slots is not None:
            vlad = slots.join(vlad_video, vlad_audio)
        else:
            vlad = torch.cat([vlad_video, vlad_audio], 1) if has_audio else vlad_video
        vs.summary("vlad", vlad)
        if vlad.dtype != torch.float32:
            vlad = vlad.float()
        return _project_gate_classify(vlad, vocab_size, cluster_size, hidden1_size, add_batch_norm, relu, gating,
                                      remove_diag, is_training, **unused_params)
# ... 89 lines not shown
```

learnablepoolingmethods_amd/ops.py:

```python
from __future__ import annotations

import ctypes as C
import os
import weakref
from typing import NamedTuple, Optional

import torch

from . import _capi
from ._capi import LPM_VLAD_NRM_RAW, LPM_VLAD_OUT_KMAJOR, LPM_VLAD_RESIDUAL, LPM_VLAD_SOFTMAX, LpmError, ptr, stream_ptr

BN_EPS = 1e-3
BN_DECAY = 0.999

VLAD_PRECISION = os.environ.get("LPM_VLAD_PRECISION", "bf16x3")
VLAD_TILES3 = os.environ.get("LPM_VLAD_TILES3", "1") != "0"
VLAD_FUSED = os.environ.get("LPM_VLAD_FUSED", "0") == "1"
PROJ_STREAM = os.environ.get("LPM_PROJ_STREAM", "1") != "0"
PROJ_DX_STREAM_MIN_N = int(os.environ.get("LPM_PROJ_DX_STREAM_MIN_N", "512"))
BN_ACT_FUSED = os.environ.get("LPM_BN_ACT_FUSED", "1") != "0"
BIAS_ACT_FUSED = os.environ.get("LPM_BIAS_ACT_FUSED", "1") != "0"
FACTORED_NORM_QUADFORM = os.environ.get("LPM_FACTORED_NORM_QUADFORM", "1") != "0"
VLAD_SOFTMAX_FUSED = os.environ.get("LPM_VLAD_SOFTMAX_FUSED", "0") == "1"
FRAME_ROW_TILES = os.environ.get("LPM_FRAME_ROW_TILES", "0") == "1"
VLAD_FUSED_DEBUG_FALLBACK = False

VLAD_KMAJOR_SCALED = os.environ.get("LPM_VLAD_KMAJOR_SCALED", "0") == "1"
VLAD_CLIP = os.environ.get("LPM_VLAD_CLIP", "1") != "0"
VLAD_CLIP16 = os.environ.get("LPM_VLAD_CLIP16", "1") != "0"
FFN_TILES = os.environ.get("LPM_FFN_TILES", "1") != "0"
DIRECT_WGRAD = True
FFN_MOD_FUSED = os.environ.get("LPM_FFN_MOD_FUSED", "1") != "0"
ASSIGN_PRECISION = os.environ.get("LPM_ASSIGN_PRECISION", "bf16x3")

MHA_PRECISION = os.environ.get("LPM_MHA_PRECISION", "bf16x3")
MHA_BN_PRECISION = os.environ.get("LPM_MHA_BN_PRECISION", "mixed")
MHA_BN_MIXED = os.environ.get("LPM_MHA_BN_MIXED", "auto,bf16x3,bf16x3")
MHA_BN_X3_MIN_KEYS = int(os.environ.get("LPM_MHA_BN_X3_MIN_KEYS", "128"))

_XT_CACHE = {}
MHA_BN_MOMENTS = os.environ.get("LPM_MHA_BN_MOMENTS", "1") != "0"
MHA_BN_ONEPASS = os.environ.get("LPM_MHA_BN_ONEPASS", "1") != "0"
LN_IMAGE = os.environ.get("LPM_LN_IMAGE", "1") != "0"
SPLIT_VECTOR = True
V2_SPLIT_COLUMNS = True
DEBUG_TAP = None

KERNEL_TIMELINE = None


class _timed:
    def __init__(self, name, dims):
        self.name, self.dims = name, dims

    def __enter__(self):
        if KERNEL_TIMELINE is not None:
            self.t0 = torch.cuda.Event(enable_timing=True)
            self.t1 = torch.cuda.Event(enable_timing=True)
            self.t0.record()
        return self

    def __exit__(self, *exc):
        if KERNEL_TIMELINE is not None:
            self.t1.record()
            KERNEL_TIMELINE.append((self.name, self.dims, self.t0, self.t1))
        return False


def _f32(t: torch.Tensor, what: str) -> torch.Tensor:
    if t.dtype != torch.float32:
        raise LpmError(f"{what}: expected float32, got {t.dtype}")
    return t


def _rows(t: torch.Tensor, what: str) -> torch.Tensor:
    _f32(t, what)
    if t.dim() != 2 or t.stride(1) != 1:
        raise LpmError(f"{what}: need a 2-D tensor with unit column stride")
    return t


def _materialised(t: torch.Tensor, what: str) -> torch.Tensor:
    c = _XT_CACHE
    if c and c.get("unmaterialised") is not None and c["base"]() is not None and t.untyped_storage().data_ptr() == c["unmaterialised"]:
        raise LpmError(f"{what}: these frames exist as bf16 operand tiles only (frame_sample_bn(storage='bf16', materialize=False))")
    return t


def _empty(shape, like):
    return torch.empty(shape, dtype=torch.float32, device=like.device)


def bn_fold(partial, nblk, C, rows, gamma, beta, moving_mean=None, moving_var=None, eps=BN_EPS, decay=BN_DECAY):
    lib = _capi.load()
    mean, var, scale, shift = (_empty((C,), partial) for _ in range(4))
    lib.check(lib._lpm_bn_fold(ptr(partial), nblk, C, rows, ptr(gamma), ptr(beta), eps, decay, ptr(mean), ptr(var),
                               ptr(scale), ptr(shift), ptr(moving_mean), ptr(moving_var), stream_ptr()), "lpm_bn_fold")
    return mean, var, scale, shift


class _BNSmall(torch.autograd.Function):

    @staticmethod
    def forward(ctx, x, gamma, beta, moving_mean, moving_var, act, mul):
        lib = _capi.load()
        x = _f32(x, "x").contiguous()
        M, C = x.shape
        mul = _f32(mul, "mul").contiguous() if mul is not None else None
        y, mean, rstd = torch.empty_like(x), _empty((C,), x), _empty((C,), x)
        lib.check(lib._lpm_bn_small_fwd(ptr(x), M, C, ptr(gamma), ptr(beta), BN_EPS, BN_DECAY, act, ptr(mul), ptr(y), ptr(mean), ptr(rstd),
                                        ptr(moving_mean), ptr(moving_var), stream_ptr()), "lpm_bn_small_fwd")
        ctx.act = act
        ctx.save_for_backward(x, gamma, beta, mean, rstd, mul)
        return y

    @staticmethod
    def backward(ctx, dy):
        lib = _capi.load()
        x, gamma, beta, mean, rstd, mul = ctx.saved_tensors
        M, C = x.shape
        dy = _f32(dy, "dy").contiguous()
        dx, dgamma, dbeta = torch.empty_like(x), _empty((C,), x), _empty((C,), x)
        dmul = torch.empty_like(x) if ctx.act == 2 else None
        lib.check(lib._lpm_bn_small_bwd(ptr(dy), ptr(x), M, C, ptr(gamma), ptr(beta), ptr(mean), ptr(rstd), ctx.act, ptr(mul), ptr(dx),
                                        ptr(dgamma), ptr(dbeta), ptr(dmul), stream_ptr()), "lpm_bn_small_bwd")
        return dx, dgamma, dbeta, None, None, None, dmul


BN_SMALL = True


def bn_small_ok(x, mul=None):
    return (BN_SMALL and x.is_cuda and x.dim() == 2 and x.dtype == torch.float32 and 1 < x.shape[0] <= 256
            and (mul is None or (mul.shape == x.shape and mul.dtype == torch.float32)))


def bn_small(x, gamma, beta, moving_mean, moving_var, act=0, mul=None):
    return _BNSmall.apply(x, gamma, beta, moving_mean, moving_var, int(act), mul)


def folded_eval_affine(gamma, beta, moving_mean, moving_var, eps=BN_EPS):
    scale = gamma * torch.rsqrt(moving_var + eps)
    return scale, beta - moving_mean * scale


def l2_normalize_rows(x):
    lib = _capi.load()
    x = _f32(x, "model_input_raw").contiguous()
    F = x.shape[-1]
    y = torch.empty_like(x)
    lib.check(lib._lpm_l2_normalize_rows(ptr(x), x.numel() // F, F, ptr(y), stream_ptr()), "lpm_l2_normalize_rows")
    return y


def dequantize_l2_normalize(q, num_frames, max_quantized_value=2.0, min_quantized_value=-2.0):
    lib = _capi.load()
    if q.dtype != torch.uint8 or q.dim() != 3:
        raise LpmError("dequantize_l2_normalize: expected a uint8 [batch, max_frames, feature] tensor")
    q = q.contiguous()
    B, MF, F = q.shape
    nf = num_frames.to(device=q.device, dtype=torch.int32).reshape(-1).contiguous()
    if nf.numel() != B:
        raise LpmError("dequantize_l2_normalize: num_frames must have one entry per clip")
    y = torch.empty((B, MF, F), dtype=torch.float32, device=q.device)
    lib.check(lib._lpm_dequantize_l2_normalize(ptr(q), ptr(nf), B, MF, F, float(max_quantized_value), float(min_quantized_value),
                                               ptr(y), stream_ptr()), "lpm_dequantize_l2_normalize")
    return y


QUANT_MAX, QUANT_MIN = 2.0, -2.0


def _check_q8_eval(raw, is_training, what):
    if raw.dtype == torch.uint8 and is_training:
        raise LpmError(f"{what}: uint8 (quantised) frames are accepted in eval mode only (is_training=False); training needs the "
                       "dequantised, L2-normalised fp32 frames (ops.dequantize_l2_normalize)")


def _frame_inputs(lib, raw, num_frames, S, what):
    nf = num_frames.to(device=raw.device, dtype=torch.int32).contiguous()
    if raw.dtype != torch.uint8:
        return _f32(raw, what).contiguous(), nf, None
    raw = raw.contiguous()
    if raw.dim() != 3:
        raise LpmError(f"{what} must be [batch, max_frames, feature]")
    B, MF, F = raw.shape
    inv = _empty((B * S,), raw)
    lib.check(lib._lpm_frame_inv_norm_q8(ptr(raw), ptr(nf), B, MF, F, S, QUANT_MAX, QUANT_MIN, ptr(inv), stream_ptr()),
              "lpm_frame_inv_norm_q8")
    return raw, nf, inv


def _frame_apply_call(lib, name, raw, inv, *args):
    if inv is None:
        lib.check(getattr(lib, "_lpm_" + name)(ptr(raw), *args), "lpm_" + name)
    else:
        lib.check(getattr(lib, "_lpm_" + name + "_q8")(ptr(raw), ptr(inv), QUANT_MAX, QUANT_MIN, *args), "lpm_" + name + "_q8")


class _FrameSampleBN(torch.autograd.Function):
    @staticmethod
    def forward(ctx, raw, num_frames, gamma, beta, moving_mean, moving_var, S, is_training, use_bn, storage="f32", materialize=True):
        lib = _capi.load()
        raw, nf, inv = _frame_inputs(lib, raw, num_frames, S, "model_input")
        if raw.dim() != 3:
            raise LpmError("model_input must be [batch, max_frames, feature]")
        B, MF, F = raw.shape
        y = _empty((B * S, F), raw)
        mean = var = None
        if use_bn:
            if is_training:
                nblk = lib._lpm_frame_stats_nblk(B, S)
                partial = _empty((nblk, 2, F), raw)
                lib.check(lib._lpm_frame_stats(ptr(raw), ptr(nf), B, MF, F, S, ptr(partial), stream_ptr()), "lpm_frame_stats")
                mean, var, scale, shift = bn_fold(partial, nblk, F, B * S, gamma, beta, moving_mean, moving_var)
            else:
                scale, shift = folded_eval_affine(gamma, beta, moving_mean, moving_var)
                scale, shift = scale.contiguous(), shift.contiguous()
        else:
            scale = shift = None
        tiles = VLAD_PRECISION == "bf16x3" and F in (1024, 1152)
        if storage == "bf16":
            if F not in (1024, 1152):
                raise LpmError("frame_sample_bn: bf16 storage needs a 1024- or 1152-wide input")
            Dv, Da = 1024, F - 1024
            nb = lambda d: torch.empty(lib._lpm_frame_tiles_bf16_bytes(B, S, d) // 4, dtype=torch.int32, device=raw.device)
            xtv, xrv = nb(Dv), nb(Dv)
            xta, xra = (nb(Da), nb(Da)) if Da else (None, None)
            _frame_apply_call(lib, "frame_apply_tiles_bf16", raw, inv, ptr(nf), B, MF, F, S, ptr(scale), ptr(shift),
                              ptr(y) if materialize else None, ptr(xtv), ptr(xrv), Dv, ptr(xta), ptr(xra), Da, stream_ptr())
            _XT_CACHE.clear()
            _XT_CACHE.update(base=weakref.ref(y), F=F, Dv=Dv, S=S, B=B, video=xtv, audio=xta, video_rows=xrv, audio_rows=xra,
                             storage="bf16", unmaterialised=None if materialize else y.untyped_storage().data_ptr())
        elif tiles:
            Dv, Da = 1024, F - 1024
            xtv = torch.empty(lib._lpm_xt_bytes(B, S, Dv) // 4, dtype=torch.int32, device=raw.device)
            xta = torch.empty(lib._lpm_xt_bytes(B, S, Da) // 4, dtype=torch.int32, device=raw.device) if Da else None
            xrv = xra = None
            if FRAME_ROW_TILES:
                xrv = torch.empty(lib._lpm_row_tiles_bytes(B, S, Dv) // 4, dtype=torch.int32, device=raw.device)
                xra = torch.empty(lib._lpm_row_tiles_bytes(B, S, Da) // 4, dtype=torch.int32, device=raw.device) if Da else None
                _frame_apply_call(lib, "frame_apply_tiles2", raw, inv, ptr(nf), B, MF, F, S, ptr(scale), ptr(shift), ptr(y), ptr(xtv),
                                  ptr(xrv), Dv, ptr(xta), ptr(xra), Da, stream_ptr())
            else:
                _frame_apply_call(lib, "frame_apply_tiles", raw, inv, ptr(nf), B, MF, F, S, ptr(scale), ptr(shift), ptr(y), ptr(xtv), Dv,
                                  ptr(xta), Da, stream_ptr())
            _XT_CACHE.clear()
            _XT_CACHE.update(base=weakref.ref(y), F=F, Dv=Dv, S=S, B=B, video=xtv, audio=xta, video_rows=xrv, audio_rows=xra)
        else:
            _frame_apply_call(lib, "frame_apply", raw, inv, ptr(nf), B, MF, F, S, ptr(scale), ptr(shift), ptr(y), stream_ptr())
        ctx.use_bn, ctx.is_training, ctx.S = use_bn, is_training, S
        ctx.q8 = inv is not None
        if use_bn and not ctx.q8:
            if is_training:
                ctx.save_for_backward(raw, nf, mean, var)
            else:
                ctx.save_for_backward(raw, nf, moving_mean.detach().clone(), moving_var.detach().clone())
        return y

    @staticmethod
    def backward(ctx, dy):
        if not ctx.use_bn:
            return (None,) * 11
        if ctx.q8:
            raise LpmError("frame_sample_bn: no gradient through the eval-mode path of uint8 frames")
        lib = _capi.load()
        raw, nf, mean, var = ctx.saved_tensors
        B, MF, F = raw.shape
        dy = _rows(dy.contiguous(), "dy")
        dgamma, dbeta = _empty((F,), raw), _empty((F,), raw)
        wsb = lib._lpm_frame_stats_workspace_bytes(B, ctx.S, F)
        ws = torch.empty(wsb // 4, dtype=torch.float32, device=raw.device)
        lib.check(lib._lpm_frame_bn_bwd(ptr(dy), dy.stride(0), ptr(raw), ptr(nf), B, MF, F, ctx.S, ptr(mean), ptr(var),
                                        BN_EPS, ptr(dgamma), ptr(dbeta), ptr(ws), wsb, stream_ptr()), "lpm_frame_bn_bwd")
        return None, None, dgamma, dbeta, None, None, None, None, None, None, None


TOPK_MAX_K = 64
TOPK_MAX_V = 65536


def topk_rows(p, k):
    if p.dtype != torch.float32 or p.dim() != 2:
        raise LpmError("topk_rows: expected a float32 [batch, classes] tensor")
    B, V = p.shape
    k = int(k)
    if not (1 <= k <= TOPK_MAX_K and k <= V <= TOPK_MAX_V):
        raise LpmError(f"topk_rows: need 1 <= k <= {TOPK_MAX_K} and k <= classes <= {TOPK_MAX_V} (k={k}, classes={V})")
    lib = _capi.load()
    p = p.contiguous()
    index = torch.empty((B, k), dtype=torch.int32, device=p.device)
    value = torch.empty((B, k), dtype=torch.float32, device=p.device)
    if B:
        lib.check(lib._lpm_topk_rows(ptr(p), B, V, k, ptr(index), ptr(value), stream_ptr()), "lpm_topk_rows")
    return index, value


class EvalRows(NamedTuple):
    hit1: torch.Tensor
    num_labels: torch.Tensor
    hits_at_n: torch.Tensor
    loss_row: Optional[torch.Tensor]
    top_index: torch.Tensor
    top_value: torch.Tensor
    top_label: torch.Tensor


def _eval_rows_out(B, k, with_loss, dev) -> EvalRows:
    return EvalRows(hit1=torch.empty(B, dtype=torch.uint8, device=dev), num_labels=torch.empty(B, dtype=torch.int32, device=dev),
                    hits_at_n=torch.empty(B, dtype=torch.int32, device=dev),
                    loss_row=torch.empty(B, dtype=torch.float64, device=dev) if with_loss else None,
                    top_index=torch.empty((B, k), dtype=torch.int32, device=dev),
                    top_value=torch.empty((B, k), dtype=torch.float32, device=dev), top_label=torch.empty((B, k), dtype=torch.uint8, device=dev))


def eval_rows(p, labels, k, with_loss=True, out: Optional[EvalRows] = None) -> EvalRows:
    if not isinstance(p, torch.Tensor) or p.dtype != torch.float32 or p.dim() != 2:
        raise LpmError("eval_rows: expected float32 predictions [batch, classes]")
    if not isinstance(labels, torch.Tensor) or labels.dtype not in (torch.uint8, torch.bool) or labels.shape != p.shape:
        raise LpmError(f"eval_rows: expected bool or uint8 labels of the predictions' shape {tuple(p.shape)}")
    B, V = p.shape
    k = int(k)
    if not (1 <= k <= TOPK_MAX_K and k <= V <= TOPK_MAX_V):
        raise LpmError(f"eval_rows: need 1 <= k <= {TOPK_MAX_K} and k <= classes <= {TOPK_MAX_V} (k={k}, classes={V})")
    if not (p.is_cuda and labels.is_cuda and p.device == labels.device):
        raise LpmError("eval_rows: predictions and labels must be on the same GPU device (eval_util.EvaluationMetrics computes the "
                       "metrics of CPU tensors)")
    if out is None:
        out = _eval_rows_out(B, k, with_loss, p.device)
    else:
        like = _eval_rows_out(0, k, out.loss_row is not None, "meta")
        for name, t, ref in zip(EvalRows._fields, out, like):
            if (t is None) != (ref is None) or (t is not None and (t.dtype != ref.dtype or t.device != p.device or not t.is_contiguous()
                                                                   or tuple(t.shape) != (B,) + tuple(ref.shape[1:]))):
                raise LpmError(f"eval_rows: out.{name} must be a contiguous {ref.dtype if ref is not None else None} tensor of "
                               f"{(B,) + tuple(ref.shape[1:]) if ref is not None else ''} on {p.device}")
    lib = _capi.load()
    p = p.contiguous()
    y = labels.contiguous()
    if y.dtype == torch.bool:
        y = y.view(torch.uint8)
    if B:
        lib.check(lib._lpm_eval_rows(ptr(p), ptr(y), B, V, k, ptr(out.hit1), ptr(out.num_labels), ptr(out.hits_at_n), ptr(out.loss_row),
                                     ptr(out.top_index), ptr(out.top_value), ptr(out.top_label), stream_ptr()), "lpm_eval_rows")
    return out


_SIDE_STREAMS = {}


class side_stream:

    def __init__(self, *inputs):
        self.inputs = [t for t in inputs if t is not None]
        self.forked = False

    def __enter__(self):
        if not self.forked:
# ... 3 lines not shown
            if dev not in _SIDE_STREAMS:
                _SIDE_STREAMS[dev] = torch.cuda.Stream(device=dev)
            self.side = _SIDE_STREAMS[dev]
            self.side.wait_stream(self.main)
            for t in self.inputs:
                t.record_stream(self.side)
            for key in ("video", "audio", "video_rows", "audio_rows"):
                t = _XT_CACHE.get(key)
                if t is not None:
                    t.record_stream(self.side)
        self.ctx = torch.cuda.stream(self.side)
        self.ctx.__enter__()
        return self

    def __exit__(self, *exc):
        return self.ctx.__exit__(*exc)

    def join(self, *outputs):
        self.main.wait_stream(self.side)
        for t in outputs:
            t.record_stream(self.main)


class _SplitColumns(torch.autograd.Function):

    @staticmethod
    def forward(ctx, x, c):
        a, b = x[:, :c], x[:, c:]
        slot = {"buf": None, "shape": tuple(x.shape), "device": x.device}
        ctx.slot, ctx.c = slot, c
        a._lpm_dx_slot, b._lpm_dx_slot = (slot, 0), (slot, c)
        return a, b

    @staticmethod
    def backward(ctx, da, db):
        slot, c = ctx.slot, ctx.c
        buf, slot["buf"] = slot["buf"], None
        M, F = slot["shape"]
        if (buf is not None and da is not None and db is not None and da.stride() == (F, 1) and db.stride() == (F, 1)
                and da.data_ptr() == buf.data_ptr() and db.data_ptr() == buf.data_ptr() + c * buf.element_size()):
            return buf, None
        if da is None:
            da = torch.zeros((M, c), dtype=torch.float32, device=slot["device"])
        if db is None:
            db = torch.zeros((M, F - c), dtype=torch.float32, device=slot["device"])
        return torch.cat([da, db], dim=1), None


class _SplitVector(torch.autograd.Function):

    @staticmethod
    def forward(ctx, v, c):
        ctx.c, ctx.n, ctx.like = c, v.shape[0], v
        return v[:c], v[c:]

    @staticmethod
    def backward(ctx, da, db):
        c, n, like = ctx.c, ctx.n, ctx.like
        if da is None:
            da = torch.zeros(c, dtype=like.dtype, device=like.device)
        if db is None:
            db = torch.zeros(n - c, dtype=like.dtype, device=like.device)
        return torch.cat([da.reshape(-1), db.reshape(-1)]), None


def split_vector(v, c):
    return _SplitVector.apply(v, int(c))


def split_columns(x, c):
    return _SplitColumns.apply(x, int(c))


def _dx_slot_view(slot_ref, D):
    if slot_ref is None:
        return None
    slot, c0 = slot_ref
    if slot["buf"] is None:
        slot["buf"] = torch.empty(slot["shape"], dtype=torch.float32, device=slot["device"])
    return slot["buf"][:, c0:c0 + D]


def frame_sample_bn(raw, num_frames, S, gamma=None, beta=None, moving_mean=None, moving_var=None, is_training=True, storage="f32",
                    materialize=True):
    _check_q8_eval(raw, is_training, "frame_sample_bn")
    use_bn = gamma is not None
    return _FrameSampleBN.apply(raw, num_frames, gamma, beta, moving_mean, moving_var, int(S), bool(is_training), use_bn, storage,
                                bool(materialize))


class _FrameSampleBNSplit(torch.autograd.Function):

    @staticmethod
    def forward(ctx, raw, num_frames, gamma, beta, moving_mean, moving_var, S, is_training, Dv):
        lib = _capi.load()
        raw, nf, inv = _frame_inputs(lib, raw, num_frames, S, "model_input")
        B, MF, F = raw.shape
        Da = F - Dv
        if is_training:
            nblk = lib._lpm_frame_stats_nblk(B, S)
            partial = _empty((nblk, 2, F), raw)
            lib.check(lib._lpm_frame_stats(ptr(raw), ptr(nf), B, MF, F, S, ptr(partial), stream_ptr()), "lpm_frame_stats")
            mean, var, scale, shift = bn_fold(partial, nblk, F, B * S, gamma, beta, moving_mean, moving_var)
        else:
            scale, shift = folded_eval_affine(gamma, beta, moving_mean, moving_var)
            scale, shift = scale.contiguous(), shift.contiguous()
            mean, var = moving_mean.detach().clone(), moving_var.detach().clone()
        yv, ya = _empty((B * S, Dv), raw), _empty((B * S, Da), raw)
        xtv = torch.empty(lib._lpm_xt_bytes(B, S, Dv) // 4, dtype=torch.int32, device=raw.device)
        xta = torch.empty(lib._lpm_xt_bytes(B, S, Da) // 4, dtype=torch.int32, device=raw.device)
        _frame_apply_call(lib, "frame_apply_tiles_split", raw, inv, ptr(nf), B, MF, F, S, ptr(scale), ptr(shift), ptr(yv), ptr(ya), ptr(xtv),
                          Dv, ptr(xta), Da, stream_ptr())
        _XT_CACHE.clear()
        _XT_CACHE.update(split=True, F=F, Dv=Dv, S=S, B=B, video=xtv, audio=xta, video_t=yv, audio_t=ya,
                         video_ver=yv._version, audio_ver=ya._version)
        ctx.S, ctx.Dv, ctx.q8 = S, Dv, inv is not None
        ctx.save_for_backward(raw, nf, mean, var)
        return yv, ya

    @staticmethod
    def backward(ctx, dv, da):
        if ctx.q8:
            raise LpmError("frame_sample_bn_split: no gradient through the eval-mode path of uint8 frames")
        lib = _capi.load()
        raw, nf, mean, var = ctx.saved_tensors
        B, MF, F = raw.shape
        Dv = ctx.Dv
        M = B * ctx.S
        dv = _rows(dv.contiguous(), "dy") if dv is not None else torch.zeros((M, Dv), dtype=torch.float32, device=raw.device)
        da = _rows(da.contiguous(), "dy") if da is not None else torch.zeros((M, F - Dv), dtype=torch.float32, device=raw.device)
        dgamma, dbeta = _empty((F,), raw), _empty((F,), raw)
        wsb = lib._lpm_frame_stats_workspace_bytes(B, ctx.S, F)
        ws = torch.empty(wsb // 4, dtype=torch.float32, device=raw.device)
        lib.check(lib._lpm_frame_bn_bwd_split(ptr(dv), dv.stride(0), ptr(da), da.stride(0), Dv, ptr(raw), ptr(nf), B, MF, F, ctx.S, ptr(mean),
                                              ptr(var), BN_EPS, ptr(dgamma), ptr(dbeta), ptr(ws), wsb, stream_ptr()), "lpm_frame_bn_bwd_split")
        return None, None, dgamma, dbeta, None, None, None, None, None


FRAME_SPLIT = os.environ.get("LPM_FRAME_SPLIT", "1") != "0"


def frame_sample_bn_split_ok(raw, Dv, is_training=True):
    dtype_ok = raw.dtype == torch.float32 or (raw.dtype == torch.uint8 and not is_training)
    return bool(FRAME_SPLIT and raw.is_cuda and raw.dim() == 3 and dtype_ok and VLAD_PRECISION == "bf16x3"
                and 0 < Dv < raw.shape[2] and Dv % 32 == 0 and (raw.shape[2] - Dv) % 32 == 0)


def frame_sample_bn_split(raw, num_frames, S, gamma, beta, moving_mean, moving_var, is_training, Dv):
    _check_q8_eval(raw, is_training, "frame_sample_bn_split")
    return _FrameSampleBNSplit.apply(raw, num_frames, gamma, beta, moving_mean, moving_var, int(S), bool(is_training), int(Dv))


_K1_CHECKED = set()
K1_SELFCHECK = os.environ.get("LPM_K1_SELFCHECK", "1") != "0"


def _k1_selfcheck(lib, planes, dev):
    if not K1_SELFCHECK or planes in _K1_CHECKED:
        return
    _K1_CHECKED.add(planes)
    import warnings
    B, T, D = 3, 120, 1024
    g = torch.Generator(device="cpu").manual_seed(20251)
    x = torch.randn(B * T, D, generator=g).to(dev)
    st = stream_ptr()
    prev = lib._lpm_k1_forms_disable(0)
    try:
        for K, bit in ((256, 1), (512, 2)) if planes == 1 else ((256, 1),):
            W = (torch.randn(D, K, generator=g) / 32).to(dev)
            nblk = lib._lpm_assign_gemm_tiles_nblk(B, T)
            if planes == 2:
# ... 197 lines not shown
def _aggregate_bwd_tiles(lib, dout, nrm, asum, colsq, csq, gsq, assign, scale, shift, x, xr, centres, B, T, D, K, flags, kmajor,
                         no_dx=False, nrm_raw=False, raw_kmajor=False):
    st = stream_ptr()
    if xr is None:
        xr = _tile_buffer(lib._lpm_row_tiles_bytes(B, T, D), x)
        lib.check(lib._lpm_split_rows_tiles(ptr(x), x.stride(0), B, T, D, ptr(xr), st), "lpm_split_rows_tiles")
    dassign = _empty((B * T, K), x)
    dcentres = _empty((D, K), x) if (centres is not None or no_dx) else None
    g0 = _empty((B, D), x) if no_dx else None
    wsb = lib._lpm_vlad_bwd_tiles_workspace_bytes(B, T, D, K)
    ws = _tile_buffer(wsb, x)
    fl = flags | (LPM_VLAD_OUT_KMAJOR if kmajor else 0) | (LPM_VLAD_NRM_RAW if nrm_raw else 0)
    if raw_kmajor:
        fl |= _capi.LPM_VLAD_RAW_KMAJOR
    dob = D * K
    if (dout.dim() == 2 and not kmajor and not raw_kmajor and dout.dtype == torch.float32 and dout.stride(1) == 1
            and dout.stride(0) >= D * K and dout.stride(0) % 4 == 0 and dout.data_ptr() % 16 == 0):
        dob = dout.stride(0)
    else:
        dout = dout.contiguous()
    with _timed("vlad_aggregate_bwd", (B, T, D, K)):
        lib.check(lib._lpm_vlad_aggregate_bwd_tiles_ld(ptr(dout), dob, ptr(nrm), ptr(asum), ptr(colsq), ptr(csq), ptr(gsq), ptr(assign),
                                                       ptr(scale), ptr(shift), ptr(xr), ptr(centres), B, T, D, K, fl, ptr(dassign),
                                                       ptr(dcentres), ptr(g0), ptr(ws), wsb, st), "lpm_vlad_aggregate_bwd_tiles")
    return dassign, dcentres, (ws, wsb), g0


def _aggregate_bwd_tiles_dx(lib, wspace, dlr, wtt, like, B, T, D, K, out=None):
    ws, wsb = wspace
    dx = out if out is not None else _empty((B * T, D), like)
    with _timed("vlad_aggregate_bwd_dx", (B, T, D, K)):
        lib.check(lib._lpm_vlad_aggregate_bwd_tiles_dx(ptr(ws), wsb, ptr(dlr), ptr(wtt), B, T, D, K, ptr(dx), dx.stride(0), 0,
                                                       stream_ptr()), "lpm_vlad_aggregate_bwd_tiles_dx")
    return dx


def _assign_gemm_dw_tiles(lib, x, xt, dl, B, T, D, K):
    st = stream_ptr()
    if xt is None:
        xt = _tile_buffer(lib._lpm_xt_bytes(B, T, D), x)
        lib.check(lib._lpm_split_frames(ptr(x), x.stride(0), B, T, D, ptr(xt), st), "lpm_split_frames")
    dlt = _tile_buffer(lib._lpm_xt_bytes(B, T, K), x)
    lib.check(lib._lpm_split_frames(ptr(dl), dl.stride(0), B, T, K, ptr(dlt), st), "lpm_split_frames")
    dW = _empty((D, K), x)
    wsb = lib._lpm_assign_gemm_tiles_bwd_dw_workspace_bytes(B, T, D, K)
    ws = _tile_buffer(max(wsb, 16), x)
    with _timed("assign_gemm_bwd_dw", (B * T, D, K)):
        lib.check(lib._lpm_assign_gemm_tiles_bwd_dw(ptr(xt), ptr(dlt), B, T, D, K, ptr(dW), ptr(ws), wsb, st),
                  "lpm_assign_gemm_tiles_bwd_dw")
    return dW


def _assign_gemm_dx_operands(lib, W, dl, B, T, D, K):
    st = stream_ptr()
    dlr = _tile_buffer(lib._lpm_row_tiles_bytes(B, T, K), dl)
    wtt = _tile_buffer(lib._lpm_weight_tiles_bytes(K, D), dl)
    lib.check(lib._lpm_split_rows_tiles(ptr(dl), dl.stride(0), B, T, K, ptr(dlr), st), "lpm_split_rows_tiles")
    lib.check(lib._lpm_split_weight_tiles(ptr(W), K, D, 1, ptr(wtt), st), "lpm_split_weight_tiles")
    return dlr, wtt


class _NetVLAD(torch.autograd.Function):

    @staticmethod
    def forward(ctx, x, W, gamma, beta, moving_mean, moving_var, bias, W2, T, is_training, kmajor, in_gamma=None, in_beta=None,
                storage="f32", lazy=False, out_slot=None):
        lib = _capi.load()
        x = _rows(x, "reshaped_input")
        W = _f32(W, "cluster_weights").contiguous()
        M, D = x.shape
        K = W.shape[1]
        if M % T:
            raise LpmError(f"rows {M} not divisible by max_frames {T}")
        B = M // T
        ctx.storage = storage
        ctx.lazy = bool(lazy)
        if out_slot is not None and storage != "bf16":
            raise LpmError("netvlad: an output slot is taken by the bf16-storage form only")
        if storage == "bf16":
            return _NetVLAD._forward_bf16(ctx, lib, x, W, gamma, beta, moving_mean, moving_var, bias, W2, B, T, D, K, is_training, kmajor,
                                          in_gamma, in_beta, out_slot, lazy)
        if storage != "f32":
            raise LpmError(f"unknown storage {storage!r} (f32 | bf16)")
        _materialised(x, "reshaped_input")
        logits = _empty((M, K), x)
        if ASSIGN_PRECISION not in ("bf16x3", "f32"):
            raise LpmError(f"unknown LPM_ASSIGN_PRECISION {ASSIGN_PRECISION!r} (bf16x3 | f32)")
        tiles = ASSIGN_PRECISION == "bf16x3" and bool(lib._lpm_assign_gemm_tiles_supported(T, D, K))
        xr = None
        if tiles:
            st = stream_ptr()
            nblk = lib._lpm_assign_gemm_tiles_nblk(B, T)
            partial = _empty((nblk, 2, K), x)
            xr = _cached_tiles(x, B, T, D, rows=True)
            if xr is None:
                xr = _tile_buffer(lib._lpm_row_tiles_bytes(B, T, D), x)
                with _timed("split_rows_tiles", (M, D)):
                    lib.check(lib._lpm_split_rows_tiles(ptr(x), x.stride(0), B, T, D, ptr(xr), st), "lpm_split_rows_tiles")
            wt = _weight_tiles(W, D, K, False, x, pack=False)
            _k1_selfcheck(lib, 2, x.device)
            with _timed("assign_gemm_fwd", (M, D, K)):
                lib.check(lib._lpm_assign_gemm_tiles_fwd(ptr(xr), ptr(wt), B, T, D, K, ptr(logits), ptr(partial), st),
                          "lpm_assign_gemm_tiles_fwd")
        else:
            nblk = lib._lpm_assign_gemm_nblk(M)
            partial = _empty((nblk, 2, K), x)
            with _timed("assign_gemm_fwd", (M, D, K)):
                lib.check(lib._lpm_assign_gemm_fwd(ptr(x), x.stride(0), ptr(W), M, D, K, 0, ptr(logits), ptr(partial),
                                                   stream_ptr()), "lpm_assign_gemm_fwd")
        mean = var = None
        use_bn = gamma is not None
        if use_bn:
            if is_training:
                mean, var, scale, shift = bn_fold(partial, nblk, K, M, gamma, beta, moving_mean, moving_var)
            else:
                scale, shift = folded_eval_affine(gamma, beta, moving_mean, moving_var)
                scale, shift = scale.contiguous(), shift.contiguous()
                mean, var = moving_mean.detach().clone(), moving_var.detach().clone()
        else:
            scale, shift = None, bias.contiguous()
        flags = LPM_VLAD_SOFTMAX | (LPM_VLAD_RESIDUAL if W2 is not None else 0)
        centres = W2.reshape(D, K).contiguous() if W2 is not None else None
        ctx.nrm_raw = _nrm_raw_ok(lib, T, D, K)
        ctx.no_dx = in_gamma is not None and tiles and _bwd_tiles_ok(lib, T, D, K)
        if lazy and not (kmajor and ctx.nrm_raw):
            raise LpmError("netvlad: the lazily normalised descriptor needs the k-major layout and the tile forms of K2 / K3")
        out, nrm, asum, colsq, csq, gsq, xt = _aggregate_fwd(lib, logits, scale, shift, x, centres, B, T, D, K, flags, kmajor,
                                                             nrm_raw=ctx.nrm_raw, save_u=any(ctx.needs_input_grad), lazy=lazy)
        ctx.dims = (B, T, D, K, flags, kmajor, use_bn, is_training, W2 is not None, tiles)
        ctx.dx_slot = getattr(x, "_lpm_dx_slot", None)
        if in_gamma is not None and not ctx.no_dx:
            raise LpmError("netvlad: the input_bn gradient shortcut needs the tile (bf16x3) forms of K1 and K3 for this shape")
        if lazy:
            rs = out._lpm_row_scale
            nrm = out.detach()
            ctx.save_for_backward(x, W, logits, scale, shift, mean, var, gamma, centres, nrm, asum, colsq, csq, gsq, xt, xr,
                                  in_gamma, in_beta)
            out._lpm_row_scale = rs
            return out
        ctx.save_for_backward(x, W, logits, scale, shift, mean, var, gamma, centres, nrm, asum, colsq, csq, gsq, xt, xr,
                              in_gamma, in_beta)
        return out

    @staticmethod
    def _forward_bf16(ctx, lib, x, W, gamma, beta, moving_mean, moving_var, bias, W2, B, T, D, K, is_training, kmajor, in_gamma, in_beta,
                      out_slot=None, lazy=False):
        st = stream_ptr()
        M = B * T
        if kmajor:
            raise LpmError("netvlad: bf16 storage writes the descriptor in the reference's d-major layout only")
        if not (lib._lpm_vlad_tiles3_supported(D, K) and lib._lpm_assign_gemm_tiles_supported(T, D, K) and K % 8 == 0):
            raise LpmError(f"netvlad: bf16 storage needs D, K multiples of 128 and K <= 512 (D={D} K={K})")
        if in_gamma is None and ctx.needs_input_grad[0]:
            raise LpmError("netvlad: bf16 storage has no input-gradient path (pass input_affine, or frames that need no gradient)")
        xr = _cached_tiles(x, B, T, D, rows=True, storage="bf16")
        xt = _cached_tiles(x, B, T, D, storage="bf16")
        if xr is None or xt is None:
            raise LpmError("netvlad: bf16 storage needs the operand tiles of ops.frame_sample_bn(storage='bf16') for this input")
        nblk = lib._lpm_assign_gemm_tiles_nblk(B, T)
        partial = _empty((nblk, 2, K), W)
        wt = _tile_buffer(lib._lpm_weight_tiles_bytes(D, K) // 2, W)
        lib.check(lib._lpm_split_weight_tiles_bf16(ptr(W), D, K, 0, ptr(wt), st), "lpm_split_weight_tiles_bf16")
        logits = torch.empty((M, K), dtype=torch.bfloat16, device=W.device)
        _k1_selfcheck(lib, 1, W.device)
        with _timed("assign_gemm_fwd", (M, D, K)):
            lib.check(lib._lpm_assign_gemm_tiles_fwd_bf16(ptr(xr), ptr(wt), B, T, D, K, ptr(logits), ptr(partial), st),
                      "lpm_assign_gemm_tiles_fwd_bf16")
# ... 2281 lines not shown
```

learnablepoolingmethods_amd/train.py:

```python
from __future__ import annotations

import contextlib
import math
import os
from typing import Dict, List, Optional

import torch
import torch.distributed as dist

from . import FLAGS, layers, losses, ops, utils
from . import variables as vs

ARENA_ALIGN = 4096

LAST_COLLECTIVE = "none yet"


def _note(what: str):
    global LAST_COLLECTIVE
    LAST_COLLECTIVE = what


def learning_rate(base_learning_rate, global_step, batch_size, num_towers, decay_examples, decay):
    p = math.floor(global_step * batch_size * num_towers / decay_examples)
# ... 348 lines not shown
                if cur != self.main_stream:
                    self.main_stream.wait_stream(cur)
                for side in ops._SIDE_STREAMS.values():
                    self.main_stream.wait_stream(side)
                self.arena.gather_names(self.bucket_names[b])
                self.sync.launch(b)
        else:
            self.arena.gather_names(self.bucket_names[b])
            self.sync.launch(b)

    def gathered_names(self):
        return {n for b in self.gathered for n in self.bucket_names[b]}


def normalize_input(raw, num_frames=None):
    if raw.dtype == torch.uint8:
        if raw.is_cuda:
            return ops.dequantize_l2_normalize(raw, num_frames)
        t = torch.arange(raw.shape[1], device=raw.device).view(1, -1, 1)
        x = torch.where(t < num_frames.view(-1, 1, 1), utils.Dequantize(raw.float()), torch.zeros((), device=raw.device))
        return layers.l2_normalize(x, 2)
    if raw.is_cuda and raw.shape[-1] % 4 == 0 and raw.shape[-1] <= 2048 and not raw.requires_grad:
        return ops.l2_normalize_rows(raw)
    return layers.l2_normalize(raw, 2)


class Trainer:

    def __init__(self, model, vocab_size=3862, batch_size=None, base_learning_rate=None, learning_rate_decay=None,
                 learning_rate_decay_examples=None, regularization_penalty=None, clip_gradient_norm=None,
                 label_loss_fn=None, device="cuda", group=None, seed=0, model_kwargs=None):
        self.model = model
        self.vocab_size = vocab_size
        self.batch_size = batch_size or FLAGS.batch_size
        self.base_lr = FLAGS.base_learning_rate if base_learning_rate is None else base_learning_rate
        self.lr_decay = FLAGS.learning_rate_decay if learning_rate_decay is None else learning_rate_decay
        self.lr_decay_examples = (FLAGS.learning_rate_decay_examples if learning_rate_decay_examples is None
                                  else learning_rate_decay_examples)
        self.reg_penalty = FLAGS.regularization_penalty if regularization_penalty is None else regularization_penalty
        self.clip = FLAGS.clip_gradient_norm if clip_gradient_norm is None else clip_gradient_norm
        self.loss_fn = label_loss_fn or losses.CrossEntropyLoss()
        self.device = torch.device(device)
        self.group = group
        self.store = vs.VariableStore(device=self.device, seed=seed)
        self.store.analytic_l2 = self.device.type == "cuda"
        self._l2_regs = []
        self.model_kwargs = dict(model_kwargs or {})
        self.global_step = 0
        self.arena: Optional[ParameterArena] = None
        self.sync: Optional[GradientSynchronizer] = None
        self.bucket_gather = None
        self.factored = None
        self.w16 = None
        self._update_stream, self._update_joined = None, True
        self._poisoned = None
        self.sharded: Optional[ShardedVariableUpdate] = None
        self.weight_pack = ops.WeightPack() if self.device.type == "cuda" else None
        self.operand_scales = None
        fp16_models = ("NetVladV1",) if os.environ.get("LPM_V2_FP16") == "0" else ("NetVladV1", "NetVladV2")
        if (self.device.type == "cuda" and FLAGS.dense_arithmetic == "fp16x2" and type(model).__name__ in fp16_models
                and os.environ.get("LPM_DENSE_ARITHMETIC", "fp16x2") == "fp16x2"):
            self.operand_scales = ops.OperandScales(self.device)
        if self.device.type == "cuda":
            ops.enable_library_gemm_selection()

    @property
    def num_towers(self) -> int:
        if dist.is_available() and dist.is_initialized():
            return dist.get_world_size(self.group)
        return 1

    def _forward(self, model_input, num_frames, labels, **kw):
        with vs.use_store(self.store):
            with vs.variable_scope("tower"):
                fused = labels is not None and type(self.loss_fn) is losses.CrossEntropyLoss
                result = self.model.create_model(model_input, num_frames=num_frames, vocab_size=self.vocab_size,
                                                 labels=labels, fused_cross_entropy=fused, **{**self.model_kwargs, **kw})
            reg_losses = self.store.pop_regularization_losses()
            self._l2_regs = self.store.pop_l2_regularizers()
        return result, reg_losses

    def _normalize_input(self, raw, num_frames=None):
        return normalize_input(raw, num_frames)

    def build(self, model_input_raw, num_frames, labels):
        if self.arena is not None:
            return
        with torch.no_grad():
            x = self._normalize_input(model_input_raw.to(self.device), num_frames.to(self.device))
            before = {n: v.clone() for n, v in self.store.vars.items() if not self.store.trainable[n]}
            self._forward(x, num_frames, labels)
            self._l2_regs = []
            for n, v in self.store.vars.items():
                if n in before:
                    v.copy_(before[n])
                elif n.endswith("/moving_mean"):
                    v.zero_()
                elif n.endswith("/moving_variance"):
                    v.fill_(1.0)
        gather = self.device.type == "cuda"
        self.arena = ParameterArena(self.store, first=["tower/hidden1_weights"], gather=gather, bucket_of=dp_bucket_of)
        bucket_names: Dict[int, List[str]] = {}
        for n in self.arena.names:
            bucket_names.setdefault(dp_bucket_of(n), []).append(n)
        ranges = []
        for b in range(4):
            names = bucket_names.get(b, [])
            if names:
                ranges.append((self.arena.segment(names[0])[0], self.arena.segment(names[-1])[1]))
            else:
                ranges.append((ranges[-1][1], ranges[-1][1]) if ranges else (0, 0))
        self.sync = GradientSynchronizer(self.arena.grad, ranges, self.group)
        early = (lambda: self.sync.launch(0)) if self.sync.active else None
        h1 = "tower/hidden1_weights"
        self.factored = None
        self.w16 = None
        self.sharded = None
        shard_from = FLAGS.hidden1_sharded_min_towers or (FLAGS.hidden1_factored_max_towers + 1)
        want_sharded = (self.sync.active and FLAGS.hidden1_sharded_update and self.num_towers >= shard_from
                        and h1 in self.arena.views and self.arena.names[0] == h1
                        and ShardedVariableUpdate.supported(self.arena, h1, self.num_towers))
        want_factored = (self.device.type == "cuda" and FLAGS.hidden1_factored_update and not want_sharded
                         and self.num_towers <= FLAGS.hidden1_factored_max_towers
                         and h1 in self.arena.views and self.arena.names[0] == h1
                         and self.arena.views[h1].dim() == 2 and self.arena.views[h1].shape[1] % 32 == 0)
        if self.sync.active:
            b = int(model_input_raw.shape[0])
            flag = torch.tensor([1 if (want_factored and b % 16 == 0) else 0, b, -b, 1 if want_sharded else 0], dtype=torch.int64,
                                device=self.device)
            _note("all_reduce(MIN) of the hidden1 gradient-route agreement (Trainer.build)")
            dist.all_reduce(flag, op=dist.ReduceOp.MIN, group=self.group)
            lo, hi = int(flag[1]), -int(flag[2])
            want_factored = bool(flag[0]) and lo == hi
            want_sharded = bool(flag[3])
        if want_sharded:
            self.sharded = ShardedVariableUpdate(self.arena, h1, self.group)
            n1 = self.arena.offsets_host[1]
            self._tail_offsets = (self.arena.offsets[1:] - n1).contiguous()
            self._tail_scratch = None
            if self.device.type == "cuda":
                self.arena.mark_direct(h1, on_ready=self._sharded_ready)
            else:
                self.arena.views[h1].register_post_accumulate_grad_hook(lambda p: self._sharded_ready())
        elif want_factored:
            self.factored = ops.FactoredGradient(on_put=self._factored_put, strict=self.sync.active)
            self.arena.views[h1]._lpm_factored = self.factored
            if FLAGS.netvlad_storage == "bf16" and FLAGS.hidden1_compute_copy and self.device.type == "cuda":
                self.w16 = ops.ComputeCopy(self.arena.views[h1], also=(self.arena.param,))
                self.arena.views[h1]._lpm_w16 = self.w16
            n1 = self.arena.offsets_host[1]
            self._tail_offsets = (self.arena.offsets[1:] - n1).contiguous()
            self._factored_scratch = self._tail_scratch = None
            self._factored_work = []
        elif self.device.type == "cuda" and h1 in self.arena.views:
            self.arena.mark_direct("tower/hidden1_weights", on_ready=early)
        if self.device.type == "cuda" and not self.sync.active and FLAGS.direct_weight_gradients:
            for n in self.arena.names:
                enc = n.endswith("/kernel") and "_attention/" in n
                moe = n in ("tower/gates/weights", "tower/experts/weights")
                if (enc or moe) and self.arena.views[n].dim() == 2 and n not in {d[0] for d in self.arena.direct}:
                    self.arena.mark_direct(n)
        if (early is not None and self.sharded is None and self.factored is None and self.device.type != "cuda"
                and h1 in self.arena.views):
            self.arena.views[h1].register_post_accumulate_grad_hook(lambda p: early())
        import os
        early_buckets = [int(b) for b in os.environ.get("LPM_DP_EARLY_BUCKETS", "1,2").split(",") if b != ""]
        self.bucket_gather = (BucketGather(self.arena, self.sync, bucket_names, early=early_buckets)
                              if (gather and self.sync.active and early_buckets) else None)
        if self.sync.active:
            _note("broadcast of the parameter arena from rank 0 (Trainer.build)")
            dist.broadcast(self.arena.param, src=0, group=self.group)
            for n, v in self.store.vars.items():
                if not self.store.trainable[n]:
                    dist.broadcast(v, src=0, group=self.group)
            self.invalidate_compute_copies()

    def _check_not_poisoned(self):
        if self._poisoned is not None:
            raise RuntimeError("this Trainer is in an inconsistent state: a step failed AFTER hidden1_weights (and its Adam moments) had "
                               "been advanced inside backward (FLAGS.hidden1_early_update) while global_step and every other variable "
                               f"stayed behind -- restore() a checkpoint or build a new Trainer.  The step failed with: {self._poisoned!r}")

    def step(self, model_input_raw, num_frames, labels, **kw):
        self._check_not_poisoned()
        self._join_update_stream()
        dev = self.device
        model_input_raw = model_input_raw.to(dev)
        labels = labels.to(dev)
        num_frames = num_frames.to(dev)
        self.build(model_input_raw, num_frames, labels)
        self.arena.zero_grad()
        if self.bucket_gather is not None:
            self.bucket_gather.arm()
        model_input = self._normalize_input(model_input_raw, num_frames)
        if self.operand_scales is not None:
            self.operand_scales.begin_step()
            ops._ACTIVE_SCALES = self.operand_scales
        if self.weight_pack is not None:
            self.weight_pack.begin_step()
            ops._ACTIVE_PACK = self.weight_pack
        try:
            return self._step_body(model_input_raw, model_input, num_frames, labels, kw)
        except BaseException as e:
            early = getattr(self, "_early", None)
            if early is not None and early.get("done"):
                self._poisoned = e
            raise
        finally:
            ops._ACTIVE_SCALES = None
            if self.weight_pack is not None:
                ops._ACTIVE_PACK = None
                self.weight_pack.end_step()

    def _step_body(self, model_input_raw, model_input, num_frames, labels, kw):
        result, reg_losses = self._forward(model_input, num_frames, labels, **kw)
        predictions = result["predictions"]
        label_loss = result["loss"] if "loss" in result else self.loss_fn.calculate_loss(predictions, labels)
        reg_loss = result.get("regularization_loss", 0.0)
        if reg_losses:
            reg_loss = reg_loss + torch.stack(reg_losses).sum()
        final_loss = self.reg_penalty * reg_loss + label_loss
        self.arena.l2 = {}
        direct = {d[0] for d in self.arena.direct}
        for w, scale in self._l2_regs:
            name = self.arena._name_of.get(id(w))
            if name is None or not self.arena.gather or (name in direct and self.sync.active):
                raise RuntimeError("analytic L2 penalty on a variable the gather-mode arena does not gather")
            self.arena.l2[name] = self.arena.l2.get(name, 0.0) + self.reg_penalty * scale
        self._l2_regs = []
        self._l2_fold = None
        fold_l2 = FLAGS.fold_l2_into_update
        if os.environ.get("LPM_L2_FOLD") in ("0", "1"):
            fold_l2 = os.environ["LPM_L2_FOLD"] == "1"
        if (self.arena.l2 and fold_l2 and self.device.type == "cuda" and not self.sync.active and self.sharded is None
                and not (self.factored is not None and self.arena.names[0] in self.arena.l2)):
            key = tuple(sorted(self.arena.l2.items()))
            if getattr(self, "_l2_key", None) != key:
                vec = torch.zeros(len(self.arena.names), dtype=torch.float32)
                for n, c in self.arena.l2.items():
                    vec[self.arena.names.index(n)] = c
                self._l2_vec, self._l2_key = vec.to(self.device), key
            self._l2_fold = self._l2_vec
            self._l2_folded = dict(self.arena.l2)
            self.arena.l2 = {}
        else:
            self._l2_folded = {}
        fg = self.factored
        if fg is not None:
            fg.clear()
            fg.armed = True
            fg.fold_dx = False
        self._early = None
        if fg is not None and not self.sync.active and FLAGS.hidden1_early_update:
            lr0 = learning_rate(self.base_lr, self.global_step, model_input_raw.shape[0], self.num_towers, self.lr_decay_examples, self.lr_decay)
            self._early = {"lr": lr0, "step": self.global_step + 1, "done": False}
            fold = FLAGS.hidden1_fold_input_gradient
            if os.environ.get("LPM_FOLD_DX") in ("0", "1"):
                fold = os.environ["LPM_FOLD_DX"] == "1"
            fg.fold_dx = bool(fold and self.w16 is not None)
        try:
            final_loss.backward()
        finally:
            if fg is not None:
                fg.armed = False
        factored = fg is not None and fg.pending
        skip = set(self.bucket_gather.gathered_names()) if self.bucket_gather is not None else set()
        if factored:
            skip.add(self.arena.names[0])
        self.arena.collect(skip=skip)
        if self.sharded is not None:
            self._sharded_ready()
        self.sync.finish()
        lr = learning_rate(self.base_lr, self.global_step, model_input_raw.shape[0], self.num_towers,
                           self.lr_decay_examples, self.lr_decay)
        self.global_step += 1
        self._l2_lr = (lr, self.global_step)
        if self.sharded is not None:
# ... 276 lines not shown
```

Baseline: 12410.

## Fuse per-frame L2 normalisation into frame sampling, BN stats and tile packing

When training NetVladV1 on fp32 frames, the separate L2-normalise pass over the raw input is skipped. A new kernel computes per-row inverse norms together with the BN statistics, and a new LDS-staged tile kernel applies the norm, BN affine and split-bf16 packing directly from raw frames, without materialising the normalised or BN'd frames. The MHA backward kernel also folds the lse and Dq subtraction into the MFMA accumulator initialisation. This cuts full-size memory passes and kernel launches. In exchange there is no explicit gradient through the unmaterialised frames, and more special-case gating on shape, alignment and precision.

```diff
diff --git a/include/lpm_hip.h b/include/lpm_hip.h
--- a/include/lpm_hip.h
+++ b/include/lpm_hip.h
@@ -67,6 +67,11 @@
                            const float* scale, const float* shift, float* y, void* xt_video, void* xr_video, int Dv,
                            void* xt_audio, void* xr_audio, int Da, lpm_stream_t stream);
 int lpm_frame_stats_nblk(int B, int S);
+int lpm_frame_stats_inv_norm(const float* raw, const int32_t* num_frames, int B, int max_frames, int F, int S, float* inv_norm,
+                             float* partial, lpm_stream_t stream);
+int lpm_frame_apply_tiles2_n(const float* raw, const float* inv_norm, const int32_t* num_frames, int B, int max_frames, int F, int S,
+                             const float* scale, const float* shift, float* y, void* xt_video, void* xr_video, int Dv,
+                             void* xt_audio, void* xr_audio, int Da, lpm_stream_t stream);
 int lpm_frame_inv_norm_q8(const unsigned char* q, const int32_t* num_frames, int B, int max_frames, int F, int S,
                           float max_quantized_value, float min_quantized_value, float* inv_norm, lpm_stream_t stream);
 int lpm_frame_apply_q8(const unsigned char* q, const float* inv_norm, float max_quantized_value, float min_quantized_value,
diff --git a/learnablepoolingmethods_amd/_capi.py b/learnablepoolingmethods_amd/_capi.py
--- a/learnablepoolingmethods_amd/_capi.py
+++ b/learnablepoolingmethods_amd/_capi.py
@@ -44,6 +44,8 @@
     "lpm_frame_bn_bwd": (_i, [_f, _l, _f, _f, _i, _i, _i, _i, _f, _f, _fl, _f, _f, _f, _s, _f]),
     "lpm_frame_bn_bwd_split": (_i, [_f, _l, _f, _l, _i, _f, _f, _i, _i, _i, _i, _f, _f, _fl, _f, _f, _f, _s, _f]),
     "lpm_frame_inv_norm_q8": (_i, [_f, _f, _i, _i, _i, _i, _fl, _fl, _f, _f]),
+    "lpm_frame_stats_inv_norm": (_i, [_f, _f, _i, _i, _i, _i, _f, _f, _f]),
+    "lpm_frame_apply_tiles2_n": (_i, [_f, _f, _f, _i, _i, _i, _i, _f, _f, _f, _f, _f, _i, _f, _f, _i, _f]),
     "lpm_frame_apply_q8": (_i, [_f, _f, _fl, _fl, _f, _i, _i, _i, _i, _f, _f, _f, _f]),
     "lpm_frame_apply_tiles_q8": (_i, [_f, _f, _fl, _fl, _f, _i, _i, _i, _i, _f, _f, _f, _f, _i, _f, _i, _f]),
     "lpm_frame_apply_tiles_split_q8": (_i, [_f, _f, _fl, _fl, _f, _i, _i, _i, _i, _f, _f, _f, _f, _f, _i, _f, _i, _f]),
diff --git a/learnablepoolingmethods_amd/csrc/frame_prep.hip b/learnablepoolingmethods_amd/csrc/frame_prep.hip
--- a/learnablepoolingmethods_amd/csrc/frame_prep.hip
+++ b/learnablepoolingmethods_amd/csrc/frame_prep.hip
@@ -27,8 +27,36 @@
     return rsqrtf(fmaxf(ss, 1e-12f));
 }
 
+__device__ __forceinline__ float row_inv_norm(const float4* __restrict__ src, int lane, int F4, float4 (&v)[8]) {
+    float ss = 0.f;
+#pragma unroll
+    for (int i = 0; i < 8; ++i) {
+#pragma clang fp contract(off)
+        const int c = lane + 64 * i;
+        v[i] = (c < F4) ? src[c] : make_float4(0.f, 0.f, 0.f, 0.f);
+        float t = v[i].x * v[i].x;
+        t = fmaf(v[i].y, v[i].y, t);
+        t = fmaf(v[i].z, v[i].z, t);
+        t = fmaf(v[i].w, v[i].w, t);
+        ss += t;
+    }
+    ss = wave_sum(ss);
+    return rsqrtf(fmaxf(ss, 1e-12f));
+}
+
+struct FrameL2 {};
 template <typename T>
 struct FrameSrc;
+template <>
+struct FrameSrc<FrameL2> {
+    const float* __restrict__ raw;
+    const float* __restrict__ inv;
+    __device__ __forceinline__ float4 load4(int64_t off, int64_t row) const {
+        const float s = inv[row];
+        const float4 v = *reinterpret_cast<const float4*>(raw + off);
+        return make_float4(__fmul_rn(v.x, s), __fmul_rn(v.y, s), __fmul_rn(v.z, s), __fmul_rn(v.w, s));
+    }
+};
 template <>
 struct FrameSrc<float> {
     const float* __restrict__ raw;
@@ -76,6 +104,53 @@
         float* p = partial + (int64_t)blockIdx.x * 2 * F;
         p[c] = s;
         p[F + c] = q;
+    }
+}
+
+constexpr int FSN_NT = 512, FSN_NW = FSN_NT / 64;
+__global__ __launch_bounds__(FSN_NT) void frame_stats_inv_norm_kernel(const float* __restrict__ raw, const int32_t* __restrict__ num_frames,
+                                                                      int B, int max_frames, int F, int S, float step,
+                                                                      float* __restrict__ inv, float* __restrict__ partial) {
+    __shared__ int64_t base[FP_ROWS];
+    __shared__ float invs[FP_ROWS];
+    const int tid = threadIdx.x, lane = tid & 63, wave = tid >> 6;
+    const int F4 = F >> 2;
+    const int r0 = blockIdx.x * FP_ROWS, rows = B * S;
+    const int nr = min(rows - r0, FP_ROWS);
+    if (tid < nr) {
+        const int r = r0 + tid, b = r / S, j = r % S;
+        int idx = sample_index(j, step, num_frames[b]);
+        idx = max(0, min(idx, max_frames - 1));
+        base[tid] = ((int64_t)b * max_frames + idx) * F;
+    }
+    __syncthreads();
+    float4 s = make_float4(0.f, 0.f, 0.f, 0.f), q = s;
+    for (int g0 = 0; g0 < nr; g0 += FSN_NW) {
+        const int ng = min(FSN_NW, nr - g0);
+        if (wave < ng) {
+            float4 v[8];
+            const float n = row_inv_norm(reinterpret_cast<const float4*>(raw + base[g0 + wave]), lane, F4, v);
+            if (lane == 0) {
+                invs[g0 + wave] = n;
+                inv[r0 + g0 + wave] = n;
+            }
+        }
+        __syncthreads();
+        if (tid < F4) {
+#pragma clang fp contract(off)
+            for (int k = 0; k < ng; ++k) {
+                const float4 v = *reinterpret_cast<const float4*>(raw + base[g0 + k] + 4 * tid);
+                const float n = invs[g0 + k];
+                const float x = __fmul_rn(v.x, n), y = __fmul_rn(v.y, n), z = __fmul_rn(v.z, n), w = __fmul_rn(v.w, n);
+                s.x += x; s.y += y; s.z += z; s.w += w;
+                q.x = fmaf(x, x, q.x); q.y = fmaf(y, y, q.y); q.z = fmaf(z, z, q.z); q.w = fmaf(w, w, q.w);
+            }
+        }
+    }
+    if (tid < F4) {
+        float4* p = reinterpret_cast<float4*>(partial + (int64_t)blockIdx.x * 2 * F);
+        p[tid] = s;
+        p[F4 + tid] = q;
     }
 }
 
@@ -358,6 +433,78 @@
     }
 }
 
+constexpr int FT_CW = 128, FT_LD = FT_CW + 8;
+template <typename Src>
+__global__ __launch_bounds__(256) void frame_apply_tiles2_lds_kernel(Src raw, const int32_t* __restrict__ num_frames, int B, int max_frames,
+                                                                     int F, int S, float step, const float* __restrict__ scale,
+                                                                     const float* __restrict__ shift, float* __restrict__ y,
+                                                                     uint4* __restrict__ xtv, uint4* __restrict__ xrv, int Dv,
+                                                                     uint4* __restrict__ xta, uint4* __restrict__ xra, int Da) {
+    __shared__ __attribute__((aligned(16))) unsigned short pl[2][32][FT_LD];
+    const int MT = 2 * ((S + 63) / 64), NSF = (S + 15) / 16;
+    const int CV = (Dv + FT_CW - 1) / FT_CW, CC = CV + (Da + FT_CW - 1) / FT_CW;
+    const int cc = blockIdx.x % CC, m = (blockIdx.x / CC) % MT, b = blockIdx.x / (CC * MT);
+    const bool video = cc < CV;
+    const int Dn = video ? Dv : Da, cb0 = (video ? cc : cc - CV) * FT_CW;
+    const int cw = min(FT_CW, Dn - cb0), c0 = (video ? 0 : Dv) + cb0;
+    uint4* __restrict__ xt = video ? xtv : xta;
+    uint4* __restrict__ xr = video ? xrv : xra;
+    const int tid = threadIdx.x, lane = tid & 63, wave = tid >> 6;
+    {
+        const int col = 4 * (tid & 31);
+        if (col < cw) {
+            float4 sc = make_float4(1.f, 1.f, 1.f, 1.f), sh = make_float4(0.f, 0.f, 0.f, 0.f);
+            if (scale) {
+                sc = *reinterpret_cast<const float4*>(scale + c0 + col);
+                sh = *reinterpret_cast<const float4*>(shift + c0 + col);
+            }
+            const int nf = num_frames[b];
+#pragma unroll
+            for (int it = 0; it < 4; ++it) {
+                const int fr = 8 * it + (tid >> 5), j = 32 * m + fr;
+                float4 f = make_float4(0.f, 0.f, 0.f, 0.f);
+                if (j < S) {
+                    int idx = sample_index(j, step, nf);
+                    idx = max(0, min(idx, max_frames - 1));
+                    const int64_t row = (int64_t)b * S + j;
+                    f = raw.load4(((int64_t)b * max_frames + idx) * F + c0 + col, row);
+                    f.x = fmaf(f.x, sc.x, sh.x); f.y = fmaf(f.y, sc.y, sh.y); f.z = fmaf(f.z, sc.z, sh.z); f.w = fmaf(f.w, sc.w, sh.w);
+                    if (y) *reinterpret_cast<float4*>(y + row * F + c0 + col) = f;
+                }
+                const float v[4] = {f.x, f.y, f.z, f.w};
+                unsigned h[4], l[4];
+#pragma unroll
+                for (int q = 0; q < 4; ++q) {
+                    h[q] = fp_bf16_rne(v[q]);
+                    l[q] = fp_bf16_rne(v[q] - __uint_as_float(h[q] << 16));
+                }
+                *reinterpret_cast<uint2*>(&pl[0][fr][col]) = make_uint2(h[0] | (h[1] << 16), h[2] | (h[3] << 16));
+                *reinterpret_cast<uint2*>(&pl[1][fr][col]) = make_uint2(l[0] | (l[1] << 16), l[2] | (l[3] << 16));
+            }
+        }
+    }
+    __syncthreads();
+    const int np = cw / 8;
+    const int CS = Dn / 16, DT = Dn / 32;
+    for (int pi = wave; pi < np; pi += 4) {
+        const int p = pi & 1;
+        {
+            const int cs = pi >> 1;
+            const uint4 t = *reinterpret_cast<const uint4*>(&pl[p][lane & 31][16 * cs + 8 * (lane >> 5)]);
+            xr[((((int64_t)b * MT + m) * CS + (cb0 >> 4) + cs) * 2 + p) * 64 + lane] = t;
+        }
+        const int dtl = (pi >> 1) % (cw / 32), stl = (pi >> 1) / (cw / 32), st = 2 * m + stl;
+        if (st < NSF) {
+            const int col = 32 * dtl + (lane & 31), f0 = 16 * stl + 8 * (lane >> 5);
+            unsigned e[8];
+#pragma unroll
+            for (int i = 0; i < 8; ++i) e[i] = pl[p][f0 + i][col];
+            xt[((((int64_t)b * NSF + st) * DT + (cb0 >> 5) + dtl) * 2 + p) * 64 + lane] =
+                make_uint4(e[0] | (e[1] << 16), e[2] | (e[3] << 16), e[4] | (e[5] << 16), e[6] | (e[7] << 16));
+        }
+    }
+}
+
 }
 
 static inline int fp_nblk(int B, int S) { return (B * S + lpm::FP_ROWS - 1) / lpm::FP_ROWS; }
@@ -432,11 +579,20 @@
         LPM_REQUIRE(xt_video && xr_video && ((scale == nullptr) == (shift == nullptr)) && ((xt_audio == nullptr) == (xr_audio == nullptr)),
                     LPM_ERR_BADARG, "%s: bad pointers", name);
     else
-        LPM_REQUIRE(y && xt_video && ((scale == nullptr) == (shift == nullptr)) && (Da == 0 || xt_audio), LPM_ERR_BADARG,
-                    "%s: bad pointers", name);
+        LPM_REQUIRE(xt_video && ((scale == nullptr) == (shift == nullptr)) && (Da == 0 || xt_audio) &&
+                        (y || (xr_video && (Da == 0 || xr_audio))), LPM_ERR_BADARG, "%s: bad pointers", name);
     LPM_REQUIRE(Dv > 0 && Da >= 0 && Dv + Da == F && Dv % 32 == 0 && Da % 32 == 0, LPM_ERR_UNSUPPORTED_SHAPE,
                 "%s: need Dv + Da == F, both multiples of 32 (F=%d Dv=%d Da=%d)", name, F, Dv, Da);
     const float step = 1.0f / (float)S;
+    if constexpr (PL == 2) {
+        if (xr_video && (Da == 0 || xr_audio) && (((uintptr_t)raw.raw | (uintptr_t)y | (uintptr_t)scale | (uintptr_t)shift) & 15) == 0) {
+            const int64_t items = (int64_t)B * 2 * ((S + 63) / 64) * ((Dv + FT_CW - 1) / FT_CW + (Da + FT_CW - 1) / FT_CW);
+            LPM_REQUIRE(items < (int64_t)1 << 31, LPM_ERR_UNSUPPORTED_SHAPE, "%s: too many work items", name);
+            hipLaunchKernelGGL(frame_apply_tiles2_lds_kernel<Src>, dim3((unsigned)items), dim3(256), 0, stream, raw, num_frames, B, max_frames, F,
+                               S, step, scale, shift, y, (uint4*)xt_video, (uint4*)xr_video, Dv, (uint4*)xt_audio, (uint4*)xr_audio, Da);
+            return check_launch(name);
+        }
+    }
     const int64_t total = (int64_t)B * 4 * ((S + 63) / 64) * 2 * (F / 8);
     const int64_t want = (total + 255) / 256;
     hipLaunchKernelGGL((frame_apply_tiles_bf16_kernel<PL, Src>), dim3((unsigned)(want < 16384 ? want : 16384)), dim3(256), 0, stream, raw,
@@ -495,6 +651,27 @@
     LPM_FRAME_CHECK("lpm_frame_apply_tiles2");
     return launch_frame_apply_tiles_bf16<2>(FrameSrc<float>{raw}, num_frames, B, max_frames, F, S, scale, shift, y, xt_video, xr_video, Dv,
                                             xt_audio, xr_audio, Da, (hipStream_t)stream, "lpm_frame_apply_tiles2");
+}
+
+extern "C" int lpm_frame_stats_inv_norm(const float* raw, const int32_t* num_frames, int B, int max_frames, int F, int S, float* inv_norm,
+                                        float* partial, lpm_stream_t stream) {
+    using namespace lpm;
+    LPM_FRAME_CHECK("lpm_frame_stats_inv_norm");
+    LPM_REQUIRE(inv_norm && partial, LPM_ERR_BADARG, "lpm_frame_stats_inv_norm: null output");
+    LPM_REQUIRE(F <= 2048 && ((uintptr_t)raw & 15) == 0 && ((uintptr_t)partial & 15) == 0, LPM_ERR_UNSUPPORTED_SHAPE,
+                "lpm_frame_stats_inv_norm: need F <= 2048, 16-byte aligned pointers (F=%d)", F);
+    hipLaunchKernelGGL(frame_stats_inv_norm_kernel, dim3(fp_nblk(B, S)), dim3(FSN_NT), 0, (hipStream_t)stream, raw, num_frames, B,
+                       max_frames, F, S, 1.0f / (float)S, inv_norm, partial);
+    return check_launch("lpm_frame_stats_inv_norm");
+}
+
+extern "C" int lpm_frame_apply_tiles2_n(const float* raw, const float* inv_norm, const int32_t* num_frames, int B, int max_frames, int F,
+                                        int S, const float* scale, const float* shift, float* y, void* xt_video, void* xr_video, int Dv,
+                                        void* xt_audio, void* xr_audio, int Da, lpm_stream_t stream) {
+    LPM_FRAME_CHECK("lpm_frame_apply_tiles2_n");
+    LPM_REQUIRE(inv_norm, LPM_ERR_BADARG, "lpm_frame_apply_tiles2_n: null inverse norms");
+    return launch_frame_apply_tiles_bf16<2>(FrameSrc<lpm::FrameL2>{raw, inv_norm}, num_frames, B, max_frames, F, S, scale, shift, y, xt_video,
+                                            xr_video, Dv, xt_audio, xr_audio, Da, (hipStream_t)stream, "lpm_frame_apply_tiles2_n");
 }
 
 extern "C" int lpm_frame_inv_norm_q8(const unsigned char* q, const int32_t* num_frames, int B, int max_frames, int F, int S,
diff --git a/learnablepoolingmethods_amd/csrc/mha_x3.hip b/learnablepoolingmethods_amd/csrc/mha_x3.hip
--- a/learnablepoolingmethods_amd/csrc/mha_x3.hip
+++ b/learnablepoolingmethods_amd/csrc/mha_x3.hip
@@ -391,6 +391,8 @@
         if (D == 16) dpart += __shfl_xor(dpart, 16, 64);
         const float dqv = dpart;
         const float lq = qok ? lse[((int64_t)b * h + hh) * L + qrow] * MX_LOG2E : INFINITY;
+        const float nlq = AFFINE ? 0.f : -lq, ndq = AFFINE ? 0.f : -dqv;
+        const f32x4 st0 = {nlq, nlq, nlq, nlq}, dp0 = {ndq, ndq, ndq, ndq};
         mx_u32x4 qb1, qb2, gb1, gb2;
         mx_col_frags<D>(qh, ql, g, qb1, qb2);
         mx_col_frags<D>(gh, gl, g, gb1, gb2);
@@ -402,9 +404,16 @@
             for (int t = 0; t < 2; ++t) {
                 const int kt = 2 * j + t;
                 const mx_u32x4 ka = mx_row_frag<D>(Kp, LP, kt, l15, g), va = mx_row_frag<D>(Vp, LP, kt, l15, g);
-                f32x4 st = {0.f, 0.f, 0.f, 0.f}, dp = {0.f, 0.f, 0.f, 0.f};
-                st = mx_mfma(ka, qb1, st);
-                dp = mx_mfma(va, gb1, dp);
+                f32x4 st, dp;
+                if constexpr (AFFINE) {
+                    st = f32x4{0.f, 0.f, 0.f, 0.f};
+                    dp = f32x4{0.f, 0.f, 0.f, 0.f};
+                    st = mx_mfma(ka, qb1, st);
+                    dp = mx_mfma(va, gb1, dp);
+                } else {
+                    st = mx_mfma(ka, qb1, st0);
+                    dp = mx_mfma(va, gb1, dp0);
+                }
                 if (D == 16) {
                     st = mx_mfma(ka, qb2, st);
                     dp = mx_mfma(va, gb2, dp);
@@ -422,8 +431,14 @@
                 }
 #pragma unroll
                 for (int r = 0; r < 4; ++r) {
-                    const float pr = __builtin_amdgcn_exp2f(z[r] - lq);
-                    float dsv = pr * (dp[r] - dqv);
+                    float pr, dsv;
+                    if constexpr (AFFINE) {
+                        pr = __builtin_amdgcn_exp2f(z[r] - lq);
+                        dsv = pr * (dp[r] - dqv);
+                    } else {
+                        pr = __builtin_amdgcn_exp2f(z[r]);
+                        dsv = pr * dp[r];
+                    }
                     if (AFFINE) {
                         const int key = kt * 16 + 4 * g + r;
                         dsv = dsv * ksc[key] - cas[key] - st[r] * cbs[key];
@@ -484,7 +499,8 @@
             reinterpret_cast<mx_u32x4*>(smem)[i] = mx_u32x4{0u, 0u, 0u, 0u};
     }
     for (int i = tid; i < LP; i += MX_DKV_NT) {
-        lses[i] = (i < L) ? lse[((int64_t)b * h + hh) * L + i] * MX_LOG2E : INFINITY;
+        const float lv = (i < L) ? lse[((int64_t)b * h + hh) * L + i] * MX_LOG2E : INFINITY;
+        lses[i] = AFFINE ? lv : -lv;
         Dq[i] = 0.f;
     }
     __syncthreads();
@@ -522,7 +538,7 @@
             }
         }
         if (NH == 2) part += __shfl_xor(part, 1, 64);
-        if (i < L * NH && (i % NH) == 0) Dq[row] = part;
+        if (i < L * NH && (i % NH) == 0) Dq[row] = AFFINE ? part : -part;
     }
     __syncthreads();
 
@@ -554,16 +570,22 @@
             for (int t = 0; t < 2; ++t) {
                 const int qt = 2 * j + t;
                 const mx_u32x4 qa = mx_row_frag<D>(Qp, LP, qt, l15, g), ga = mx_row_frag<D>(Gp, LP, qt, l15, g);
-                f32x4 st = {0.f, 0.f, 0.f, 0.f}, dp = {0.f, 0.f, 0.f, 0.f};
-                st = mx_mfma(qa, kb1, st);
-                dp = mx_mfma(ga, vb1, dp);
+                const f32x4 lq4 = *reinterpret_cast<const f32x4*>(lses + qt * 16 + 4 * g);
+                const f32x4 dq4 = *reinterpret_cast<const f32x4*>(Dq + qt * 16 + 4 * g);
+                f32x4 st, dp;
+                if constexpr (AFFINE) {
+                    st = f32x4{0.f, 0.f, 0.f, 0.f};
+                    dp = f32x4{0.f, 0.f, 0.f, 0.f};
+                    st = mx_mfma(qa, kb1, st);
+                    dp = mx_mfma(ga, vb1, dp);
+                } else {
+                    st = mx_mfma(qa, kb1, lq4);
+                    dp = mx_mfma(ga, vb1, dq4);
+                }
                 if (D == 16) {
                     st = mx_mfma(qa, kb2, st);
                     dp = mx_mfma(ga, vb2, dp);
                 }
-                const float4 lq4v = *reinterpret_cast<const float4*>(lses + qt * 16 + 4 * g);
-                const float4 dq4v = *reinterpret_cast<const float4*>(Dq + qt * 16 + 4 * g);
-                const float lq4[4] = {lq4v.x, lq4v.y, lq4v.z, lq4v.w}, dq4[4] = {dq4v.x, dq4v.y, dq4v.z, dq4v.w};
 #pragma unroll
                 for (int r = 0; r < 4; ++r) {
                     const int qr = qt * 16 + 4 * g + r;
@@ -571,8 +593,8 @@
                     float z = sraw;
                     if (AFFINE) z = fmaf(sraw, sck, shk) * MX_LOG2E;
                     if (!kok) z = -INFINITY;
-                    const float pr = __builtin_amdgcn_exp2f(z - lq4[r]);
-                    const float dz = pr * (dp[r] - dq4[r]);
+                    const float pr = __builtin_amdgcn_exp2f(AFFINE ? z - lq4[r] : z);
+                    const float dz = pr * (AFFINE ? dp[r] - dq4[r] : dp[r]);
                     float dsv = dz;
                     if (AFFINE) {
                         zs += dz;
diff --git a/learnablepoolingmethods_amd/frame_level_models.py b/learnablepoolingmethods_amd/frame_level_models.py
--- a/learnablepoolingmethods_amd/frame_level_models.py
+++ b/learnablepoolingmethods_amd/frame_level_models.py
@@ -117,10 +117,11 @@
                           "switched off, the input gradient is formed explicitly from now on")
 
 
-def _sample_and_normalise(model_input, num_frames, iterations, add_batch_norm, is_training, storage="f32"):
+def _sample_and_normalise(model_input, num_frames, iterations, add_batch_norm, is_training, storage="f32", normalize=False):
     bn = layers.bn_variables("input_bn", model_input.shape[2], model_input.device) if add_batch_norm else (None,) * 4
     return ops.frame_sample_bn(model_input, num_frames.reshape(-1), iterations, *bn, is_training=is_training, storage=storage,
-                               materialize=storage == "f32" or vs.default_store().summaries is not None)
+                               materialize=(storage == "f32" or vs.default_store().summaries is not None) and not normalize,
+                               normalize=normalize)
 
 
 class NetVladV1(models.BaseModel):
@@ -157,7 +158,13 @@
                               "back to fp32 storage (explicit input-gradient path)")
             storage = "f32"
 
-        reshaped_input = _sample_and_normalise(model_input, num_frames, iterations, add_batch_norm, is_training, storage)
+        normalize = False
+        if ops.is_raw_frames(model_input):
+            normalize = bool(shortcut and storage == "f32" and feature_size in (1024, 1152) and ops.VLAD_PRECISION == "bf16x3"
+                             and vs.default_store().summaries is None and model_input.dtype == torch.float32)
+            if not normalize:
+                model_input = ops.l2_normalize_rows(model_input)
+        reshaped_input = _sample_and_normalise(model_input, num_frames, iterations, add_batch_norm, is_training, storage, normalize)
         if storage == "f32" or vs.default_store().summaries is not None:
             vs.summary("input_bn", reshaped_input)
 
diff --git a/learnablepoolingmethods_amd/ops.py b/learnablepoolingmethods_amd/ops.py
--- a/learnablepoolingmethods_amd/ops.py
+++ b/learnablepoolingmethods_amd/ops.py
@@ -23,6 +23,7 @@
 FACTORED_NORM_QUADFORM = os.environ.get("LPM_FACTORED_NORM_QUADFORM", "1") != "0"
 VLAD_SOFTMAX_FUSED = os.environ.get("LPM_VLAD_SOFTMAX_FUSED", "0") == "1"
 FRAME_ROW_TILES = os.environ.get("LPM_FRAME_ROW_TILES", "0") == "1"
+FRAME_PREP_FUSED = os.environ.get("LPM_FRAME_PREP_FUSED", "1") != "0"
 VLAD_FUSED_DEBUG_FALLBACK = False
 
 VLAD_KMAJOR_SCALED = os.environ.get("LPM_VLAD_KMAJOR_SCALED", "0") == "1"
@@ -81,10 +82,27 @@
 
 
 def _materialised(t: torch.Tensor, what: str) -> torch.Tensor:
+    if _unmaterialised(t):
+        if _XT_CACHE.get("storage") == "bf16":
+            raise LpmError(f"{what}: these frames exist as bf16 operand tiles only (frame_sample_bn(storage='bf16', materialize=False))")
+        raise LpmError(f"{what}: these frames exist as operand tiles only (frame_sample_bn(normalize=True))")
+    return t
+
+
+def _unmaterialised(t: torch.Tensor) -> bool:
     c = _XT_CACHE
-    if c and c.get("unmaterialised") is not None and c["base"]() is not None and t.untyped_storage().data_ptr() == c["unmaterialised"]:
-        raise LpmError(f"{what}: these frames exist as bf16 operand tiles only (frame_sample_bn(storage='bf16', materialize=False))")
-    return t
+    return bool(c and c.get("unmaterialised") is not None and c["base"]() is not None
+                and t.untyped_storage().data_ptr() == c["unmaterialised"])
+
+
+def raw_frames(x: torch.Tensor) -> torch.Tensor:
+    v = x.detach()
+    v._lpm_raw_frames = True
+    return v
+
+
+def is_raw_frames(x) -> bool:
+    return bool(getattr(x, "_lpm_raw_frames", False))
 
 
 def _empty(shape, like):
@@ -200,13 +218,38 @@
 
 class _FrameSampleBN(torch.autograd.Function):
     @staticmethod
-    def forward(ctx, raw, num_frames, gamma, beta, moving_mean, moving_var, S, is_training, use_bn, storage="f32", materialize=True):
+    def forward(ctx, raw, num_frames, gamma, beta, moving_mean, moving_var, S, is_training, use_bn, storage="f32", materialize=True,
+                normalize=False):
         lib = _capi.load()
         raw, nf, inv = _frame_inputs(lib, raw, num_frames, S, "model_input")
         if raw.dim() != 3:
             raise LpmError("model_input must be [batch, max_frames, feature]")
         B, MF, F = raw.shape
         y = _empty((B * S, F), raw)
+        ctx.normalize = bool(normalize)
+        if normalize:
+            if not (use_bn and is_training and storage == "f32" and inv is None and VLAD_PRECISION == "bf16x3" and F in (1024, 1152)
+                    and raw.data_ptr() % 16 == 0):
+                raise LpmError("frame_sample_bn(normalize=True): training-mode input_bn over fp32 frames of 1024 or 1152 features with "
+                               "the split-bf16 tile forms only")
+            nblk = lib._lpm_frame_stats_nblk(B, S)
+            partial = _empty((nblk, 2, F), raw)
+            inv = _empty((B * S,), raw)
+            lib.check(lib._lpm_frame_stats_inv_norm(ptr(raw), ptr(nf), B, MF, F, S, ptr(inv), ptr(partial), stream_ptr()),
+                      "lpm_frame_stats_inv_norm")
+            mean, var, scale, shift = bn_fold(partial, nblk, F, B * S, gamma, beta, moving_mean, moving_var)
+            Dv, Da = 1024, F - 1024
+            xtv = torch.empty(lib._lpm_xt_bytes(B, S, Dv) // 4, dtype=torch.int32, device=raw.device)
+            xrv = torch.empty(lib._lpm_row_tiles_bytes(B, S, Dv) // 4, dtype=torch.int32, device=raw.device)
+            xta = torch.empty(lib._lpm_xt_bytes(B, S, Da) // 4, dtype=torch.int32, device=raw.device) if Da else None
+            xra = torch.empty(lib._lpm_row_tiles_bytes(B, S, Da) // 4, dtype=torch.int32, device=raw.device) if Da else None
+            lib.check(lib._lpm_frame_apply_tiles2_n(ptr(raw), ptr(inv), ptr(nf), B, MF, F, S, ptr(scale), ptr(shift), None, ptr(xtv),
+                                                    ptr(xrv), Dv, ptr(xta), ptr(xra), Da, stream_ptr()), "lpm_frame_apply_tiles2_n")
+            _XT_CACHE.clear()
+            _XT_CACHE.update(base=weakref.ref(y), F=F, Dv=Dv, S=S, B=B, video=xtv, audio=xta, video_rows=xrv, audio_rows=xra,
+                             unmaterialised=y.untyped_storage().data_ptr())
+            ctx.use_bn, ctx.is_training, ctx.S, ctx.q8 = use_bn, is_training, S, False
+            return y
         mean = var = None
         if use_bn:
             if is_training:
@@ -260,8 +303,11 @@
 
     @staticmethod
     def backward(ctx, dy):
+        if ctx.normalize:
+            raise LpmError("frame_sample_bn(normalize=True): input_bn's gradients come from the pooling ops in closed form "
+                           "(ops.netvlad(input_affine=...)); there is no explicit gradient path through the unmaterialised frames")
         if not ctx.use_bn:
-            return (None,) * 11
+            return (None,) * 12
         if ctx.q8:
             raise LpmError("frame_sample_bn: no gradient through the eval-mode path of uint8 frames")
         lib = _capi.load()
@@ -273,7 +319,7 @@
         ws = torch.empty(wsb // 4, dtype=torch.float32, device=raw.device)
         lib.check(lib._lpm_frame_bn_bwd(ptr(dy), dy.stride(0), ptr(raw), ptr(nf), B, MF, F, ctx.S, ptr(mean), ptr(var),
                                         BN_EPS, ptr(dgamma), ptr(dbeta), ptr(ws), wsb, stream_ptr()), "lpm_frame_bn_bwd")
-        return None, None, dgamma, dbeta, None, None, None, None, None, None, None
+        return None, None, dgamma, dbeta, None, None, None, None, None, None, None, None
 
 
 TOPK_MAX_K = 64
@@ -443,11 +489,11 @@
 
 
 def frame_sample_bn(raw, num_frames, S, gamma=None, beta=None, moving_mean=None, moving_var=None, is_training=True, storage="f32",
-                    materialize=True):
+                    materialize=True, normalize=False):
     _check_q8_eval(raw, is_training, "frame_sample_bn")
     use_bn = gamma is not None
     return _FrameSampleBN.apply(raw, num_frames, gamma, beta, moving_mean, moving_var, int(S), bool(is_training), use_bn, storage,
-                                bool(materialize))
+                                bool(materialize), bool(normalize))
 
 
 class _FrameSampleBNSplit(torch.autograd.Function):
@@ -811,7 +857,10 @@
                                           in_gamma, in_beta, out_slot, lazy)
         if storage != "f32":
             raise LpmError(f"unknown storage {storage!r} (f32 | bf16)")
-        _materialised(x, "reshaped_input")
+        if not (in_gamma is not None and VLAD_PRECISION == "bf16x3" and ASSIGN_PRECISION == "bf16x3"
+                and lib._lpm_assign_gemm_tiles_supported(T, D, K) and _bwd_tiles_ok(lib, T, D, K)
+                and _cached_tiles(x, B, T, D, rows=True) is not None and _cached_tiles(x, B, T, D) is not None):
+            _materialised(x, "reshaped_input")
         logits = _empty((M, K), x)
         if ASSIGN_PRECISION not in ("bf16x3", "f32"):
             raise LpmError(f"unknown LPM_ASSIGN_PRECISION {ASSIGN_PRECISION!r} (bf16x3 | f32)")
diff --git a/learnablepoolingmethods_amd/train.py b/learnablepoolingmethods_amd/train.py
--- a/learnablepoolingmethods_amd/train.py
+++ b/learnablepoolingmethods_amd/train.py
@@ -454,6 +454,13 @@
 
     def _normalize_input(self, raw, num_frames=None):
         return normalize_input(raw, num_frames)
+
+    def _step_input(self, raw, num_frames):
+        if (ops.FRAME_PREP_FUSED and type(self.model).__name__ == "NetVladV1" and raw.is_cuda and raw.dtype == torch.float32
+                and raw.dim() == 3 and raw.shape[-1] in (1024, 1152) and raw.is_contiguous() and raw.data_ptr() % 16 == 0
+                and not raw.requires_grad):
+            return ops.raw_frames(raw)
+        return self._normalize_input(raw, num_frames)
 
     def build(self, model_input_raw, num_frames, labels):
         if self.arena is not None:
@@ -564,7 +571,7 @@
         self.arena.zero_grad()
         if self.bucket_gather is not None:
             self.bucket_gather.arm()
-        model_input = self._normalize_input(model_input_raw, num_frames)
+        model_input = self._step_input(model_input_raw, num_frames)
         if self.operand_scales is not None:
             self.operand_scales.begin_step()
             ops._ACTIVE_SCALES = self.operand_scales
```

Result: faster. 12570, median of 6 (+1.3%).
